# atx/padne

Hardware: AMD Instinct MI355X
Metric: CG solves/s (higher is better)
Workload: dtype f64; 1 GPU; C4 8-layer N=10M: 8-layer jittered triangular Laplacian, 9999392 nodes, via-ring stitched, 1 A source/sink, amg-PCG to rtol 1e-12; n_unknowns=9999391, nnz_per_rank=69955225, rows_per_rank=9999391, parallelism=layer-partitioned x1

## Files before the change

### padne_amd/csrc/amg.hip

```cpp
#include "common.hpp"

#include <functional>
#include <type_traits>
#include <memory>

#include <algorithm>
#include <chrono>
#include <math.h>
#include <stdlib.h>
#include <string.h>

namespace padne {

struct AmgLevel {
    const padne_csr *A = nullptr;
    padne_csr *A_owned = nullptr;
    padne_csr *P = nullptr;
    padne_csr *R = nullptr;
    padne_csr *W = nullptr;
    double lambda = 2.0;
    double jac = 0.0;
    long long n = 0;
    double *b = nullptr, *xa = nullptr, *xb = nullptr, *tmp = nullptr;
    float *b8 = nullptr, *xa8 = nullptr, *xb8 = nullptr, *tmp8 = nullptr;
// ... 27 lines not shown
};

constexpr double kTheta = 0.08;
constexpr double kOmegaNum = 1.5;
constexpr double kChebRatio = 10.0;
constexpr int kLanczosSteps = 8;
constexpr int kMaxLevels = 16;

struct __attribute__((packed, aligned(4))) I4u { int x, y, z, w; };
struct __attribute__((packed, aligned(4))) I2u { int x, y; };
struct __attribute__((packed, aligned(4))) D2u { double x, y; };
struct __attribute__((packed, aligned(4))) L2u { long long x, y; };
__device__ __forceinline__ int4 load_i4_unaligned(const int *p) {
    const I4u v = *reinterpret_cast<const I4u *>(p);
    return make_int4(v.x, v.y, v.z, v.w);
}
__device__ __forceinline__ double2 load_d2_unaligned(const double *p) {
    const D2u v = *reinterpret_cast<const D2u *>(p);
    return make_double2(v.x, v.y);
}

template <int LANES>
__device__ __forceinline__ int scan_incl_lanes(int x) {
    x += __builtin_amdgcn_update_dpp(0, x, 0x111, 0xf, 0xf, false);
    x += __builtin_amdgcn_update_dpp(0, x, 0x112, 0xf, 0xf, false);
    x += __builtin_amdgcn_update_dpp(0, x, 0x114, 0xf, 0xf, false);
    x += __builtin_amdgcn_update_dpp(0, x, 0x118, 0xf, 0xf, false);
    if (LANES >= 32) x += __builtin_amdgcn_update_dpp(0, x, 0x142, 0xa, 0xf, false);
    if (LANES == 64) x += __builtin_amdgcn_update_dpp(0, x, 0x143, 0xc, 0xf, false);
    return x;
}

__device__ __forceinline__ unsigned xcd_bid() {
    const unsigned b = blockIdx.x, per = gridDim.x >> 3;
    if (b >= (per << 3)) return b;
    return (b & 7u) * per + (b >> 3);
}
struct XcdSweep { long long t0, t1, stride; };
__device__ __forceinline__ XcdSweep xcd_sweep(const long long n_tiles, const int waves_per_block, const int w) {
    const unsigned G = gridDim.x;
    const unsigned nslab = (G % kNumXcd == 0) ? kNumXcd : 1;
    const unsigned slab = blockIdx.x % nslab;
    XcdSweep sw;
    const long long s0 = (long long)slab * n_tiles / nslab;
    sw.t1 = (long long)(slab + 1) * n_tiles / nslab;
    sw.t0 = s0 + (long long)(blockIdx.x / nslab) * waves_per_block + w;
    sw.stride = (long long)(G / nslab) * waves_per_block;
    return sw;
}



constexpr unsigned int kMisRoot = 0xffffffffu;
__device__ __forceinline__ unsigned int prio32_of(int i) {
    unsigned int h = (unsigned int)i & 0x7fffffffu;
    h = (h * 0x5bd1e995u) & 0x7fffffffu;
    h ^= h >> 15;
    h = (h * 0x2c1b3c6du) & 0x7fffffffu;
    h ^= h >> 13;
    h = (h * 0x297a2d39u) & 0x7fffffffu;
    h ^= h >> 16;
    return h + 1u;
}

__device__ __forceinline__ bool strong(double a, double di, double dj, double theta2) {
    return a * a * di * dj >= theta2;
}

__device__ __forceinline__ int xw_position(const int4 d, const int run, const int c) {
    int pos = 0;
    if (c >= d.z && c < d.z + run) pos = 2 * run + (c - d.z);
    if (c >= d.y && c < d.y + run) pos = run + (c - d.y);
    if (c >= d.x && c < d.x + run) pos = c - d.x;
    return pos;
}

__global__ __launch_bounds__(256) void strength_mark(int n, int n_wtiles, const int *__restrict__ rowptr,
                                                     const int *__restrict__ cols, const double *__restrict__ vals,
                                                     const double *__restrict__ dinv, double theta2,
                                                     int *__restrict__ scol, double *__restrict__ bound_partial,
                                                     const int4 *__restrict__ xw_desc = nullptr,
                                                     const unsigned char *__restrict__ xw_lidx = nullptr,
                                                     const int xw_run = 0, unsigned char *__restrict__ spos = nullptr,
                                                     float *__restrict__ vals32 = nullptr) {
    constexpr int CH = 512;
    __shared__ unsigned char rid_all[4 * CH];
    __shared__ double pv_all[4 * CH];
    __shared__ double red[4], red2[4];
    const int lane = threadIdx.x & 63, w = threadIdx.x >> 6;
    unsigned char *rid = rid_all + w * CH;
    double *pv = pv_all + w * CH;
    const XcdSweep sw = xcd_sweep(n_wtiles, 4, w);
    double my_max = 0.0, my_plain = 0.0;
    for (long long wt = sw.t0; wt < sw.t1; wt += sw.stride) {
        const int row0 = (int)wt * 64;
        const int row1 = min(row0 + 64, n);
        const int r = row0 + lane;
        int rs = 0, re = 0;
        double di = 0.0;
        if (r < row1) {
            rs = rowptr[r];
            re = rowptr[r + 1];
            di = dinv[r];
        }
        const int k0 = __shfl(rs, 0, 64);
        const int k1 = __shfl(re, row1 - row0 - 1, 64);
        double dF = r < row1 ? 1.0 / di : 1.0, off_strong = 0.0, off_all = 0.0, abs_all = 0.0;
        int4 dsc = make_int4(0, 0, 0, 0);
        if (spos != nullptr) dsc = xw_desc[wt];
        const bool windowed = spos != nullptr && dsc.w != 0;
        const int self_pos = windowed ? xw_position(dsc, xw_run, r) : 0;
        for (int base = k0; base < k1; base += CH) {
            const int lo = max(rs, base), hi = min(re, base + CH);
            for (int k = lo; k < hi; ++k) rid[k - base] = (unsigned char)lane;
            asm volatile("s_waitcnt lgkmcnt(0)" ::: "memory");
            __builtin_amdgcn_wave_barrier();
#pragma unroll
            for (int q = 0; q < CH / 64; ++q) {
                const int e = base + lane + 64 * q;
                const int rl = e < k1 ? rid[e - base] : 0;
                const double dr = __shfl(di, rl, 64);
                const int sp = __shfl(self_pos, rl, 64);
                if (e < k1) {
                    const int i = row0 + rl;
                    const int c = cols[e];
                    const double v = vals[e];
                    if (vals32 != nullptr) vals32[e] = (float)v;
                    const bool st = c != i && strong(v, dr, dinv[c], theta2);
                    scol[e] = st ? c : i;
                    if (windowed) spos[e] = st ? xw_lidx[e] : (unsigned char)sp;
                    if (bound_partial != nullptr) {
                        rid[e - base] = (unsigned char)(rl | (c == i ? 0x40 : 0) | (st ? 0x80 : 0));
                        pv[e - base] = v;
                    }
                }
            }
            if (bound_partial != nullptr) {
                asm volatile("s_waitcnt lgkmcnt(0)" ::: "memory");
                __builtin_amdgcn_wave_barrier();
                for (int k = lo; k < hi; ++k) {
                    const unsigned char f = rid[k - base];
                    const double v = pv[k - base];
                    abs_all += fabs(v);
                    if (f & 0x40) continue;
                    off_all += fabs(v);
                    if (f & 0x80) off_strong += fabs(v);
                    else dF += v;
                }
            }
            asm volatile("" ::: "memory");
            __builtin_amdgcn_wave_barrier();
        }
        if (bound_partial != nullptr && r < row1) {
            double off = off_strong;
            if (!(dF * di > 0.05)) {
                dF = 1.0 / di;
                off = off_all;
            }
            const double sgm = (off + fabs(dF)) / fabs(dF);
            my_max = sgm > my_max ? sgm : my_max;
            const double plain = abs_all * fabs(di);
            my_plain = plain > my_plain ? plain : my_plain;
        }
    }
    if (bound_partial != nullptr) {
        for (int o = 32; o > 0; o >>= 1) {
            my_max = fmax(my_max, __shfl_down(my_max, o, 64));
            my_plain = fmax(my_plain, __shfl_down(my_plain, o, 64));
        }
        if (lane == 0) {
            red[w] = my_max;
            red2[w] = my_plain;
        }
        __syncthreads();
        if (threadIdx.x == 0) {
            bound_partial[blockIdx.x] = fmax(fmax(red[0], red[1]), fmax(red[2], red[3]));
            bound_partial[kMaxPartials + blockIdx.x] = fmax(fmax(red2[0], red2[1]), fmax(red2[2], red2[3]));
        }
    }
}

template <typename T>
__global__ __launch_bounds__(256) void nbr_max(int n, int n_wtiles, const int *__restrict__ srow,
                                               const int *__restrict__ scol, const T *__restrict__ in,
                                               T *__restrict__ out) {
    constexpr int CH = 512;
    __shared__ T park_all[4 * CH];
    const int lane = threadIdx.x & 63, w = threadIdx.x >> 6;
    T *park = park_all + w * CH;
    const XcdSweep sw = xcd_sweep(n_wtiles, 4, w);
    for (long long wt = sw.t0; wt < sw.t1; wt += sw.stride) {
        const int row0 = (int)wt * 64;
        const int row1 = min(row0 + 64, n);
        const int r = row0 + lane;
        int rs = 0, re = 0;
        T m = 0;
        if (r < row1) {
            rs = srow[r];
            re = srow[r + 1];
            m = in[r];
        }
        const int k0 = __shfl(rs, 0, 64);
        const int k1 = __shfl(re, row1 - row0 - 1, 64);
        for (int base = k0; base < k1; base += CH) {
#pragma unroll
            for (int j = 0; j < CH / 64; ++j) {
                const int e = base + lane + 64 * j;
                park[lane + 64 * j] = (e < k1) ? in[scol[e]] : (T)0;
            }
            asm volatile("s_waitcnt lgkmcnt(0)" ::: "memory");
            __builtin_amdgcn_wave_barrier();
            const int lo = max(rs, base), hi = min(re, base + CH);
            for (int k = lo; k < hi; ++k) {
                const T v = park[k - base];
                m = v > m ? v : m;
            }
            asm volatile("" ::: "memory");
            __builtin_amdgcn_wave_barrier();
        }
        if (r < row1) out[r] = m;
    }
}

template <typename T>
__global__ __launch_bounds__(256) void nbr_max_wpr(int n, const int *__restrict__ srow, const int *__restrict__ scol,
                                                   const T *__restrict__ in, T *__restrict__ out) {
    const int lane = threadIdx.x & 63;
    const long long r = (long long)blockIdx.x * 4 + (threadIdx.x >> 6);
    if (r >= n) return;
    const int rs = srow[r], re = srow[r + 1];
    T m = in[r];
    for (int k = rs + lane; k < re; k += 64) {
        const T v = in[scol[k]];
// ... 714 lines not shown
                    }
                    cols[s0 + b + 1] = c;
                    vals[s0 + b + 1] = v;
                }
            }
            continue;
        }
        for (int e = threadIdx.x; e < n; e += 256) {
            Cs[e] = cols[s0 + e];
            Vs[e] = vals[s0 + e];
        }
        __syncthreads();
        for (int e = threadIdx.x; e < n; e += 256) {
            const int c = Cs[e];
            int rank = 0;
            for (int f = 0; f < n; ++f) rank += Cs[f] < c ? 1 : 0;
            cols[s0 + rank] = c;
            vals[s0 + rank] = Vs[e];
        }
        __syncthreads();
    }
}

__global__ void spgemm_count(int n_rows, const int *__restrict__ xr, const int *__restrict__ xc,
                             const int *__restrict__ yr, const int *__restrict__ ye, int *__restrict__ cnt) {
    const int i = xcd_bid() * blockDim.x + threadIdx.x;
    if (i >= n_rows) return;
    long long c = 0;
    const int k0 = xr[i], k1 = xr[i + 1];
    {
        const int4 ca = load_i4_unaligned(xc + k0), cb = load_i4_unaligned(xc + k0 + 4);
        const int m[8] = {ca.x, ca.y, ca.z, ca.w, cb.x, cb.y, cb.z, cb.w};
        int ln[8];
#pragma unroll
        for (int u = 0; u < 8; ++u) {
            ln[u] = 0;
            if (k0 + u < k1) {
                if (ye == yr + 1) {
                    const I2u be = *reinterpret_cast<const I2u *>(yr + m[u]);
                    ln[u] = be.y - be.x;
                } else {
                    ln[u] = ye[m[u]] - yr[m[u]];
                }
            }
        }
#pragma unroll
        for (int u = 0; u < 8; ++u) c += ln[u];
    }
    for (int k = k0 + 8; k < k1; ++k) {
        const int m = xc[k];
        c += ye[m] - yr[m];
    }
    cnt[i] = c > 2000000000LL ? 2000000000 : (int)c;
}

template <int LPR>
__global__ __launch_bounds__(256) void spgemm_count_lanes(int n_rows, const int *__restrict__ xr, const int *__restrict__ xc,
                                                          const int *__restrict__ yr, const int *__restrict__ ye, int *__restrict__ cnt) {
    const long long tid = (long long)xcd_bid() * blockDim.x + threadIdx.x;
    const long long i = tid / LPR;
    const int l = (int)(tid % LPR);
    long long c = 0;
    if (i < n_rows) {
        const int k0 = xr[i], k1 = xr[i + 1];
        int k = k0 + l;
        for (; k + LPR < k1; k += 2 * LPR) {
            const int m0 = xc[k], m1 = xc[k + LPR];
            const int b0 = yr[m0], e0 = ye[m0], b1 = yr[m1], e1 = ye[m1];
            c += (e0 - b0) + (e1 - b1);
        }
        if (k < k1) {
            const int m0 = xc[k];
            c += ye[m0] - yr[m0];
        }
    }
#pragma unroll
    for (int d = 1; d < LPR; d <<= 1) c += __shfl_xor(c, d, 64);
    if (i < n_rows && l == 0) cnt[i] = c > 2000000000LL ? 2000000000 : (int)c;
}

__global__ void spgemm_rows(int n_rows, const int *__restrict__ xr, const int *__restrict__ xc,
                            const double *__restrict__ xv, const int *__restrict__ yr, const int *__restrict__ yc,
                            const double *__restrict__ yv, const int *__restrict__ ye, const int ycs, const int *__restrict__ slot_ptr,
                            long long *__restrict__ key, double *__restrict__ val, int *__restrict__ row_len) {
    const int i = blockIdx.x * blockDim.x + threadIdx.x;
    if (i >= n_rows) return;
    long long *K = key + slot_ptr[i];
    double *V = val + slot_ptr[i];
    int m = 0;
    for (int k = xr[i]; k < xr[i + 1]; ++k) {
        const int mid = xc[k];
        const double a = xv[k];
        for (int q = yr[mid]; q < ye[mid]; ++q) {
            const long long c = (long long)yc[(long long)q * ycs] << 32;
            const double v = a * yv[q];
            int lo = 0, hi = m;
            while (lo < hi) {
                const int h = (lo + hi) >> 1;
                if (K[h] < c) lo = h + 1; else hi = h;
            }
            if (lo < m && K[lo] == c) {
                V[lo] += v;
            } else {
                for (int t = m; t > lo; --t) {
                    K[t] = K[t - 1];
                    V[t] = V[t - 1];
                }
                K[lo] = c;
                V[lo] = v;
                ++m;
            }
        }
    }
    row_len[i] = m;
}

template <int CAP, int KC, int QC, int YCS>
__global__ __launch_bounds__(128) void spgemm_rows_lds_pipe(int n_rows, const int *__restrict__ xr, const int *__restrict__ xc,
                                                            const double *__restrict__ xv, const int *__restrict__ yr,
                                                            const int *__restrict__ yc, const double *__restrict__ yv,
                                                            const int *__restrict__ ye, const int *__restrict__ slot_ptr,
                                                            long long *__restrict__ key, double *__restrict__ val,
                                                            int *__restrict__ row_len, int *__restrict__ begin) {
    static_assert(CAP % 2 == 0, "keys are kept in pairs");
    __shared__ int2 Kc[CAP / 2][128];
    __shared__ double Vc[CAP][128];
    const int t = threadIdx.x;
    const int i = xcd_bid() * 128 + t;
    const bool live = i < n_rows;
    if (begin == nullptr && !live) return;
    int m = 0;
    bool overflow = false;
#pragma unroll
    for (int u = 0; u < CAP / 2; ++u) Kc[u][t] = make_int2(-1, -1);
    auto insert = [&](const bool act, const int c, const double v) {
        int pos = -1;
#pragma unroll
        for (int u = 0; u < CAP; u += 2) {
            if (__all(u >= m)) break;
            const int2 kk = Kc[u >> 1][t];
            pos = kk.x == c ? u : pos;
            pos = kk.y == c ? u + 1 : pos;
        }
        if (act && !overflow) {
            const bool found = pos >= 0;
            if (!found && m == CAP) {
                overflow = true;
            } else {
                const int p = found ? pos : m;
                const double base = found ? Vc[p][t] : -0.0;
                Vc[p][t] = base + v;
                if (!found) {
                    reinterpret_cast<int *>(&Kc[p >> 1][t])[p & 1] = c;
                    ++m;
                }
            }
        }
    };
    const int x0 = live ? xr[i] : 0, x1 = live ? xr[i + 1] : 0;
    for (int kb = x0; kb < x1 && !overflow; kb += KC) {
        const int nk = min(KC, x1 - kb);
        int mid[KC], ys[KC], ln[KC];
        double a[KC];
        static_assert(KC % 4 == 1 && QC == 4, "the loads below are written for 4 k + 1 entries of X and rows of Y read four at a time");
#pragma unroll
        for (int u = 0; u < KC - 1; u += 4) {
            const I4u c4 = *reinterpret_cast<const I4u *>(xc + kb + u);
            mid[u] = c4.x; mid[u + 1] = c4.y; mid[u + 2] = c4.z; mid[u + 3] = c4.w;
            const D2u v0 = *reinterpret_cast<const D2u *>(xv + kb + u), v1 = *reinterpret_cast<const D2u *>(xv + kb + u + 2);
            a[u] = v0.x; a[u + 1] = v0.y; a[u + 2] = v1.x; a[u + 3] = v1.y;
        }
        mid[KC - 1] = xc[kb + KC - 1];
        a[KC - 1] = xv[kb + KC - 1];
#pragma unroll
        for (int u = 0; u < KC; ++u) {
            mid[u] = u < nk ? mid[u] : 0;
            if (ye == yr + 1) {
                const I2u be = *reinterpret_cast<const I2u *>(yr + mid[u]);
                ys[u] = be.x;
                ln[u] = u < nk ? be.y - be.x : 0;
            } else {
                ys[u] = yr[mid[u]];
                ln[u] = u < nk ? ye[mid[u]] - ys[u] : 0;
            }
        }
        int cb[2][QC];
        double vb[2][QC];
        auto fetch = [&](const int u, int (&c)[QC], double (&v)[QC]) {
            if (YCS == 1) {
                const I4u c4 = *reinterpret_cast<const I4u *>(yc + ys[u]);
                c[0] = c4.x; c[1] = c4.y; c[2] = c4.z; c[3] = c4.w;
            } else {
                const L2u k0 = *reinterpret_cast<const L2u *>(reinterpret_cast<const long long *>(yc) + ys[u]);
                const L2u k1 = *reinterpret_cast<const L2u *>(reinterpret_cast<const long long *>(yc) + ys[u] + 2);
                c[0] = (int)k0.x; c[1] = (int)k0.y; c[2] = (int)k1.x; c[3] = (int)k1.y;
            }
            const D2u v0 = *reinterpret_cast<const D2u *>(yv + ys[u]), v1 = *reinterpret_cast<const D2u *>(yv + ys[u] + 2);
            v[0] = v0.x; v[1] = v0.y; v[2] = v1.x; v[3] = v1.y;
        };
        fetch(0, cb[0], vb[0]);
#pragma unroll
        for (int u = 0; u < KC; ++u) {
            if (u + 1 < KC) fetch(u + 1, cb[(u + 1) & 1], vb[(u + 1) & 1]);
#pragma unroll
            for (int w = 0; w < QC; ++w)
                if (__any(w < ln[u])) insert(w < ln[u], cb[u & 1][w], a[u] * vb[u & 1][w]);
            for (int q = QC; q < ln[u] && !overflow; ++q)
                insert(true, yc[(long long)(ys[u] + q) * YCS], a[u] * yv[ys[u] + q]);
        }
    }
    int place = live ? slot_ptr[i] : 0;
    if (begin != nullptr) {
        const int lane = t & 63;
        const int tile0 = i - lane, tile1 = min(tile0 + 64, n_rows);
        const int len = (live && !overflow) ? m : 0;
        const int bound = (live && overflow) ? slot_ptr[i + 1] - slot_ptr[i] : 0;
        const int incl = scan_incl_lanes<64>(len);
        const int bound_incl = scan_incl_lanes<64>(bound);
        const int back = __builtin_amdgcn_readlane(bound_incl, 63) - bound_incl + bound;
        if (tile0 < n_rows) {
            const int r_begin = slot_ptr[tile0], r_end = slot_ptr[tile1];
            place = overflow ? r_end - back : r_begin + (incl - len);
        }
        if (live) begin[i] = place;
    }
    if (!live) return;
    if (overflow) {
        row_len[i] = -1;
        return;
    }
    long long *K = key + place;
    double *V = val + place;
    int kr[CAP];
#pragma unroll
    for (int u = 0; u < CAP; u += 2) {
        const int2 kk = Kc[u >> 1][t];
        kr[u] = u < m ? kk.x : 2147483647;
        kr[u + 1] = u + 1 < m ? kk.y : 2147483647;
    }
#pragma unroll
    for (int u = 0; u < CAP; ++u) {
        if (__all(u >= m)) break;
        int rank = 0;
#pragma unroll
        for (int w = 0; w < CAP; ++w) rank += kr[w] < kr[u] ? 1 : 0;
        if (u < m) {
            K[rank] = (long long)kr[u] << 32;
            V[rank] = Vc[u][t];
        }
    }
    row_len[i] = m;
}

template <int CAPP, int HT, int LANES>
struct SpgemmRowLds {
    using Mask = typename std::conditional<LANES == 64, unsigned long long, unsigned>::type;
    int ht[HT];
    int hidx[HT];
    int dk[HT / 2];
    Mask mask[HT / 2];
    double pvb[LANES];
    double xs[LANES];
    int ys[LANES];
    int offc[LANES];
    unsigned long long bits[CAPP / 64];
};

template <int CAPP, int HT, int LANES>
__device__ __forceinline__ int spgemm_row_by_masks(SpgemmRowLds<CAPP, HT, LANES> &S, const int sl, const int sub,
                                                   const bool has_row, const int nx, const int len, const int ystart,
                                                   const double a, const int *__restrict__ yc, const double *__restrict__ yv,
                                                   const int ycs, long long *__restrict__ K, double *__restrict__ V) {
    using Mask = typename SpgemmRowLds<CAPP, HT, LANES>::Mask;
    static_assert(CAPP % 64 == 0 && CAPP / 64 <= LANES && 64 % LANES == 0, "bits of the product offsets");
    constexpr int NC = (HT / 2 + LANES - 1) / LANES;
    constexpr int EMPTY = -1;
    const unsigned long long sub_mask = (LANES == 64 ? ~0ull : ((1ull << LANES) - 1ull));
    const int shift = sub * LANES;
    const unsigned long long below = (1ull << sl) - 1ull;
    static_assert(LANES == 16 || LANES == 32 || LANES == 64, "the scan below");
    const int incl = scan_incl_lanes<LANES>(len);
    const int np = LANES == 64   ? __builtin_amdgcn_readlane(incl, 63)
                   : LANES == 32 ? (sub != 0 ? __builtin_amdgcn_readlane(incl, 63) : __builtin_amdgcn_readlane(incl, 31))
                                 : __builtin_amdgcn_update_dpp(0, incl, 0x15F, 0xf, 0xf, false);
    const bool live = has_row && nx <= LANES && np <= CAPP;
    const unsigned long long have = (__ballot(live && len > 0) >> shift) & sub_mask;
    if (live) {
        for (int h = sl; h < HT; h += LANES) S.ht[h] = EMPTY;
        for (int h = sl; h < HT / 2; h += LANES) S.mask[h] = (Mask)0;
        if (sl < CAPP / 64) S.bits[sl] = 0ull;
        asm volatile("s_waitcnt lgkmcnt(0)" ::: "memory");
        if (len > 0) {
            const int pos = __popcll(have & below);
            const int o = incl - len;
            S.offc[pos] = o;
            S.ys[pos] = ystart;
            S.xs[pos] = a;
            atomicOr(&S.bits[o >> 6], 1ull << (o & 63));
        }
    }
    asm volatile("s_waitcnt lgkmcnt(0)" ::: "memory");
    __builtin_amdgcn_wave_barrier();
    int np_w = live ? np : 0;
    if (LANES == 64) {
        np_w = __builtin_amdgcn_readfirstlane(np_w);
    } else {
        int m = 0;
#pragma unroll
        for (int g = 0; g < 64 / LANES; ++g) m = max(m, __builtin_amdgcn_readlane(np_w, g * LANES));
        np_w = m;
    }
    int cnt = 0, pre = 0;
    bool overflow = false;
// ... 5 lines not shown
        const bool mine = live && p < np;
        unsigned long long word = 0ull;
        if (live && base < np) word = S.bits[base >> 6];
        int c = 0;
        if (mine) {
            const int kk = pre + __popcll(word & (~0ull >> (63 - (p & 63)))) - 1;
            const int q = S.ys[kk] + (p - S.offc[kk]);
            c = yc[(long long)q * ycs];
            S.pvb[sl] = S.xs[kk] * yv[q];
        }
        if (((base + LANES) & 63) == 0) pre += __popcll(word);
        bool pending = mine;
        unsigned h = ((unsigned)c * 2654435761u) >> 7;
        int idx = -1;
        for (int round = 0; __any(pending); ++round) {
            if (round == HT) {
                overflow = overflow || pending;
                break;
            }
            h &= (HT - 1);
            int old = EMPTY - 1;
            if (pending) old = atomicCAS(&S.ht[h], EMPTY, c);
            const bool won = old == EMPTY;
            const unsigned long long wm = (__ballot(won) >> shift) & sub_mask;
            if (won) {
                idx = cnt + __popcll(wm & below);
                S.hidx[h] = idx;
                if (idx < HT / 2) S.dk[idx] = c;
            }
            cnt += __popcll(wm);
            asm volatile("" ::: "memory");
            const bool hit = pending && old == c;
            if (hit) idx = S.hidx[h];
            pending = pending && !won && !hit;
            ++h;
        }
        if (mine && idx >= 0 && idx < HT / 2) atomicOr(&S.mask[idx], (Mask)1 << sl);
        asm volatile("s_waitcnt lgkmcnt(0)" ::: "memory");
        __builtin_amdgcn_wave_barrier();
#pragma unroll
        for (int u = 0; u < NC; ++u) {
            const int j = sl + u * LANES;
            if (live && j < cnt && j < HT / 2) {
                Mask m = S.mask[j];
                if (m != (Mask)0) {
                    S.mask[j] = (Mask)0;
                    do {
                        const int b = (LANES == 64 ? __ffsll((long long)m) : __ffs((int)m)) - 1;
                        acc[u] += S.pvb[b];
                        m &= m - (Mask)1;
                    } while (m != (Mask)0);
                }
            }
        }
        asm volatile("s_waitcnt lgkmcnt(0)" ::: "memory");
        __builtin_amdgcn_wave_barrier();
    }
    const bool any_overflow = ((__ballot(overflow) >> shift) & sub_mask) != 0ull;
    const int nd = cnt;
    const bool ok = live && !any_overflow && nd <= HT / 2;
#pragma unroll
    for (int u = 0; u < NC; ++u) {
        const int j = sl + u * LANES;
        if (ok && j < nd) {
            const int kq = S.dk[j];
            int rank = 0;
            for (int t = 0; t < nd; ++t) rank += S.dk[t] < kq ? 1 : 0;
            K[rank] = (long long)kq << 32;
            V[rank] = acc[u];
        }
    }
    asm volatile("s_waitcnt lgkmcnt(0)" ::: "memory");
    __builtin_amdgcn_wave_barrier();
    return ok ? nd : -1;
}

template <int CAPP, int HT, int LANES, bool LIST>
__global__ __launch_bounds__(256) void spgemm_rows_lanes(int n_rows, const int *__restrict__ xr, const int *__restrict__ xc,
                                                         const double *__restrict__ xv, const int *__restrict__ yr,
                                                         const int *__restrict__ yc, const double *__restrict__ yv, const int *__restrict__ ye, const int ycs,
                                                         const int *__restrict__ slot_ptr, long long *__restrict__ key,
                                                         double *__restrict__ val, int *__restrict__ row_len,
                                                         const int *__restrict__ row_list = nullptr,
                                                         const int *__restrict__ list_count = nullptr) {
    constexpr int G = 256 / LANES;
    __shared__ SpgemmRowLds<CAPP, HT, LANES> s_rows[G];
    const int lane = threadIdx.x & 63;
    const int sl = lane % LANES, sub = lane / LANES, g = threadIdx.x / LANES;
    constexpr bool listed = LIST;
    int t_l, t_end, stride;
    if (listed) {
        t_end = *list_count;
        t_l = (int)blockIdx.x * G + g;
        stride = (int)gridDim.x * G;
    } else {
        const int nslab = (gridDim.x % kNumXcd == 0) ? kNumXcd : 1;
        const int slab = blockIdx.x % nslab;
        t_end = (int)((long long)(slab + 1) * n_rows / nslab);
        t_l = (int)((long long)slab * n_rows / nslab) + (int)(blockIdx.x / nslab) * G + g;
        stride = (int)(gridDim.x / nslab) * G;
    }
    if (t_l > t_end) t_l = t_end;
    int row_l = -1;
    int row_a = -1, x0_a = 0, x1_a = 0, len_a = -1;
    int row_b = -1, x0_b = 0, x1_b = 0, len_b = -1, mid_b = 0;
    double a_b = 0.0;
    int row_c = -1, nx_c = 0, len_c = -1, ys_c = 0, ye_c = 0, place_c = 0;
    double a_c = 0.0;
    auto advance = [&]() {
        const int nx_b = x1_b - x0_b;
        row_c = row_b; nx_c = nx_b; len_c = len_b; a_c = a_b; ys_c = 0; ye_c = 0; place_c = 0;
        if (row_b >= 0) {
            place_c = slot_ptr[row_b];
            if (nx_b <= LANES && sl < nx_b) {
                ys_c = yr[mid_b];
                ye_c = ye[mid_b];
            }
        }
        const int nx_a = x1_a - x0_a;
        row_b = row_a; x0_b = x0_a; x1_b = x1_a; len_b = len_a; mid_b = 0; a_b = 0.0;
        if (row_a >= 0 && nx_a <= LANES && sl < nx_a) {
            mid_b = xc[x0_a + sl];
            a_b = xv[x0_a + sl];
        }
        row_a = row_l; x0_a = 0; x1_a = 0; len_a = -1;
        if (row_a >= 0) {
            x0_a = xr[row_a];
            x1_a = xr[row_a + 1];
            if (listed) len_a = row_len[row_a];
        }
        row_l = -1;
        if (t_l < t_end) row_l = listed ? row_list[t_l] : t_l;
        t_l = t_l < t_end - stride ? t_l + stride : t_end;
    };
    advance();
    advance();
    advance();
    advance();
    while (__any(row_c >= 0)) {
        const int i = row_c;
        const bool has_row = i >= 0 && !(listed && len_c >= 0);
        const int nx = nx_c, ystart = ys_c, len = ye_c - ys_c, place = place_c;
        const double a = a_c;
        advance();
        const int nd = spgemm_row_by_masks<CAPP, HT, LANES>(s_rows[g], sl, sub, has_row, nx, len, ystart, a, yc, yv, ycs,
                                                            key + place, val + place);
        if (has_row && sl == 0) row_len[i] = nd;
    }
}

__global__ __launch_bounds__(256) void spgemm_rows_dense(int n_cols, const int *__restrict__ xr, const int *__restrict__ xc,
                                                         const double *__restrict__ xv, const int *__restrict__ yr,
                                                         const int *__restrict__ yc, const double *__restrict__ yv, const int *__restrict__ ye, const int ycs,
                                                         const int *__restrict__ slot_ptr, long long *__restrict__ key,
                                                         double *__restrict__ val, int *__restrict__ row_len,
                                                         const int only_pending, const int *__restrict__ row_list = nullptr,
                                                         const int *__restrict__ list_count = nullptr) {
    extern __shared__ double acc_and_flag[];
    double *acc = acc_and_flag;
    unsigned char *hit = (unsigned char *)(acc + n_cols);
    __shared__ int wave_cnt[4];
    const int n_turns = row_list != nullptr ? *list_count : 1;
    for (int turn = row_list != nullptr ? (int)blockIdx.x : 0; turn < n_turns; turn += row_list != nullptr ? (int)gridDim.x : 1) {
    const int i = row_list != nullptr ? row_list[turn] : (int)blockIdx.x;
    if (only_pending && row_len[i] >= 0) continue;
    __syncthreads();
    for (int c = threadIdx.x; c < n_cols; c += 256) {
        acc[c] = 0.0;
        hit[c] = 0;
    }
    __syncthreads();
    for (int k = xr[i]; k < xr[i + 1]; ++k) {
        const int mid = xc[k];
        const double a = xv[k];
        for (int q = yr[mid] + threadIdx.x; q < ye[mid]; q += 256) {
            const int c = yc[(long long)q * ycs];
            acc[c] += a * yv[q];
            hit[c] = 1;
        }
        __syncthreads();
    }
    long long *K = key + slot_ptr[i];
    double *V = val + slot_ptr[i];
    int base = 0;
    const int lane = threadIdx.x & 63, w = threadIdx.x >> 6;
    for (int c0 = 0; c0 < n_cols; c0 += 256) {
        const int c = c0 + threadIdx.x;
        const bool on = c < n_cols && hit[c];
        const unsigned long long bal = __ballot(on);
        if (lane == 0) wave_cnt[w] = __popcll(bal);
        __syncthreads();
        int off = base;
        for (int u = 0; u < w; ++u) off += wave_cnt[u];
        const int total = wave_cnt[0] + wave_cnt[1] + wave_cnt[2] + wave_cnt[3];
        if (on) {
            const int pos = off + __popcll(bal & ((1ull << lane) - 1ull));
            K[pos] = (long long)c << 32;
            V[pos] = acc[c];
        }
        base += total;
        __syncthreads();
    }
    if (threadIdx.x == 0) row_len[i] = base;
    }
}

__global__ __launch_bounds__(256) void collect_pending_rows(int n, const int *__restrict__ row_len, int *__restrict__ list,
                                                            int *__restrict__ count) {
    const int i = blockIdx.x * 256 + threadIdx.x;
    const bool pend = i < n && row_len[i] < 0;
    __shared__ int wave_cnt[4], block_base;
    const unsigned long long mask = __ballot(pend);
    const int lane = threadIdx.x & 63, w = threadIdx.x >> 6;
    if (lane == 0) wave_cnt[w] = __popcll(mask);
    __syncthreads();
    if (threadIdx.x == 0) {
        const int t = wave_cnt[0] + wave_cnt[1] + wave_cnt[2] + wave_cnt[3];
        block_base = t ? atomicAdd(count, t) : 0;
    }
    __syncthreads();
    int base = block_base;
    for (int q = 0; q < w; ++q) base += wave_cnt[q];
    if (pend) list[base + __popcll(mask & ((1ull << lane) - 1ull))] = i;
}

__global__ void spgemm_rows_redo(int n_rows, const int *__restrict__ xr, const int *__restrict__ xc,
                                 const double *__restrict__ xv, const int *__restrict__ yr, const int *__restrict__ yc,
                                 const double *__restrict__ yv, const int *__restrict__ ye, const int ycs, const int *__restrict__ slot_ptr,
                                 long long *__restrict__ key, double *__restrict__ val, int *__restrict__ row_len) {
    const int i = blockIdx.x * blockDim.x + threadIdx.x;
    if (i >= n_rows || row_len[i] >= 0) return;
    long long *K = key + slot_ptr[i];
    double *V = val + slot_ptr[i];
    int m = 0;
    for (int k = xr[i]; k < xr[i + 1]; ++k) {
        const int mid = xc[k];
        const double a = xv[k];
        for (int q = yr[mid]; q < ye[mid]; ++q) {
            const long long c = (long long)yc[(long long)q * ycs] << 32;
            const double v = a * yv[q];
            int lo = 0, hi = m;
            while (lo < hi) {
                const int h = (lo + hi) >> 1;
                if (K[h] < c) lo = h + 1; else hi = h;
            }
            if (lo < m && K[lo] == c) {
                V[lo] += v;
            } else {
                for (int u = m; u > lo; --u) {
                    K[u] = K[u - 1];
                    V[u] = V[u - 1];
                }
                K[lo] = c;
                V[lo] = v;
                ++m;
            }
        }
    }
    row_len[i] = m;
}

__global__ void dense_from_csr(int n, const int *__restrict__ rowptr, const int *__restrict__ cols,
                               const double *__restrict__ vals, double *__restrict__ W) {
    const int i = blockIdx.x;
    for (int c = threadIdx.x; c < n; c += blockDim.x) W[(size_t)i * n + c] = 0.0;
    __syncthreads();
    for (int k = rowptr[i] + threadIdx.x; k < rowptr[i + 1]; k += blockDim.x) W[(size_t)i * n + cols[k]] = vals[k];
}

constexpr int kGjBlock = 16;
constexpr int kGjStrip = 32;
__device__ __forceinline__ double Rsel(const double (&R)[kGjBlock], int a) {
    double v = 0.0;
#pragma unroll
    for (int b = 0; b < kGjBlock; ++b) v = (a == b) ? R[b] : v;
    return v;
}
__device__ __forceinline__ void gj_invert_block16(double (&dd)[4], const int lane) {
    const int eb = lane & 15, ea0 = lane >> 4;
#pragma unroll
    for (int p = 0; p < kGjBlock; ++p) {
        const double dpp = __shfl(dd[p >> 2], ((p & 3) << 4) | p, 64);
        const double drow = __shfl(dd[p >> 2], ((p & 3) << 4) | eb, 64);
        double dcol[4];
#pragma unroll
        for (int q = 0; q < 4; ++q) dcol[q] = __shfl(dd[q], (lane & 48) | p, 64);
        double inv = __builtin_amdgcn_rcp(dpp);
        inv = fma(inv, fma(-dpp, inv, 1.0), inv);
        inv = fma(inv, fma(-dpp, inv, 1.0), inv);
        const double rp = drow * inv;
#pragma unroll
        for (int q = 0; q < 4; ++q) {
            const int ea = ea0 + 4 * q;
            const double cp = dcol[q];
            dd[q] = (ea == p) ? (eb == p ? inv : rp) : (eb == p ? -cp * inv : dd[q] - cp * rp);
        }
    }
}

template <bool kFull>
__global__ __launch_bounds__(256) void gj_block_step(int n, int k0, const double *__restrict__ in, double *__restrict__ out) {
    static_assert(kGjBlock == 16, "the pivot block inversion below maps a 16 x 16 block onto one wave");
    __shared__ __attribute__((aligned(16))) double Dinv[kGjBlock][kGjBlock];
    __shared__ __attribute__((aligned(16))) double Lcol[kGjStrip][kGjBlock];
    const int bs = kFull ? kGjBlock : min(kGjBlock, n - k0);
    const int r0 = blockIdx.y * kGjStrip;
    const int c = blockIdx.x * blockDim.x + threadIdx.x;
    const bool live = c < n;
    const bool pivot_col = c >= k0 && c < k0 + bs;
    double P[kGjBlock], V[kGjStrip];
#pragma unroll
    for (int b = 0; b < kGjBlock; ++b) P[b] = (live && !pivot_col && b < bs) ? in[(size_t)(k0 + b) * n + c] : 0.0;
#pragma unroll
    for (int q = 0; q < kGjStrip; ++q) {
        const int i = r0 + q;
        V[q] = (live && i < n && !pivot_col) ? in[(size_t)i * n + c] : 0.0;
    }
    for (int t = threadIdx.x; t < kGjStrip * kGjBlock; t += 256) {
        const int i = r0 + t / kGjBlock, b = t % kGjBlock;
        Lcol[t / kGjBlock][b] = (i < n && (kFull || b < bs)) ? in[(size_t)i * n + k0 + b] : 0.0;
    }
    if (threadIdx.x < 64) {
        const int lane = threadIdx.x, eb = lane & 15, ea0 = lane >> 4;
        double dd[4];
#pragma unroll
        for (int q = 0; q < 4; ++q) {
            const int ea = ea0 + 4 * q;
            dd[q] = (ea < bs && eb < bs) ? in[(size_t)(k0 + ea) * n + k0 + eb] : (ea == eb ? 1.0 : 0.0);
        }
        gj_invert_block16(dd, lane);
#pragma unroll
        for (int q = 0; q < 4; ++q) Dinv[ea0 + 4 * q][eb] = dd[q];
    }
    __syncthreads();
    if (!live) return;
    double R[kGjBlock];
    if (pivot_col) {
#pragma unroll
        for (int a = 0; a < kGjBlock; ++a) R[a] = Dinv[a][c - k0];
    } else {
#pragma unroll
        for (int a = 0; a < kGjBlock; ++a) {
// ... 358 lines not shown
}

__global__ __launch_bounds__(256) void fold_range_kernel(const double *__restrict__ mins, const double *__restrict__ maxs, int g,
                                                         double *__restrict__ out2) {
    __shared__ double lo_s[256], hi_s[256];
    double lo = 1e300, hi = 0.0;
    for (int q = threadIdx.x; q < g; q += 256) {
        const double a = mins[q], b = maxs[q];
        lo = a < lo ? a : lo;
        if (b > hi || !(b == b)) hi = b;
    }
    lo_s[threadIdx.x] = lo;
    hi_s[threadIdx.x] = hi;
    __syncthreads();
    for (int off = 128; off > 0; off >>= 1) {
        if ((int)threadIdx.x < off) {
            const double a = lo_s[threadIdx.x + off], b = hi_s[threadIdx.x + off];
            if (a < lo_s[threadIdx.x]) lo_s[threadIdx.x] = a;
            if (!(hi_s[threadIdx.x] == hi_s[threadIdx.x])) {
            } else if (b > hi_s[threadIdx.x] || !(b == b)) {
                hi_s[threadIdx.x] = b;
            }
        }
        __syncthreads();
    }
    if (threadIdx.x == 0) {
        out2[0] = lo_s[0];
        out2[1] = hi_s[0];
    }
}


static bool amg_verbose();

__global__ __launch_bounds__(256) void fold_max2_kernel(const double *__restrict__ a, const double *__restrict__ b, int g,
                                                        double *__restrict__ out2) {
    __shared__ double red[2][256];
    double ma = 0.0, mb = 0.0;
    for (int q = threadIdx.x; q < g; q += 256) {
        ma = a[q] > ma ? a[q] : ma;
        if (b != nullptr) mb = b[q] > mb ? b[q] : mb;
    }
    red[0][threadIdx.x] = ma;
    red[1][threadIdx.x] = mb;
    __syncthreads();
    for (int off = 128; off > 0; off >>= 1) {
        if ((int)threadIdx.x < off) {
            red[0][threadIdx.x] = fmax(red[0][threadIdx.x], red[0][threadIdx.x + off]);
            red[1][threadIdx.x] = fmax(red[1][threadIdx.x], red[1][threadIdx.x + off]);
        }
        __syncthreads();
    }
    if (threadIdx.x == 0) {
        out2[0] = red[0][0];
        out2[1] = red[1][0];
    }
}

static int gershgorin(padne_ctx *ctx, const padne_csr *A, double *lambda, bool filtered = false) {
    const int g = (int)std::min<long long>((A->n_rows + 255) / 256, 1024);
    double *part = ctx->partials + 6 * kMaxPartials;
    if (filtered)
        hipLaunchKernelGGL(gershgorin_filtered_kernel, dim3(g > 0 ? g : 1), dim3(256), 0, ctx->stream, (int)A->n_rows,
                           A->rowptr, A->cols, A->vals, A->dinv, kTheta * kTheta, part);
    else
        hipLaunchKernelGGL(gershgorin_kernel, dim3(g > 0 ? g : 1), dim3(256), 0, ctx->stream, (int)A->n_rows, A->rowptr,
                           A->vals, A->dinv, part);
    hipLaunchKernelGGL(fold_max2_kernel, dim3(1), dim3(256), 0, ctx->stream, (const double *)part, (const double *)nullptr,
                       g > 0 ? g : 1, part + kMaxPartials - 2);
    PADNE_HIP_CHECK(hipGetLastError());
    double h[2] = {0.0, 0.0};
    PADNE_TRY(read_back(ctx, part + kMaxPartials - 2, sizeof(h), h));
    double m = h[0];
    if (!(m > 0.0) || !(m < 1e6)) m = 2.0;
    *lambda = m;
    return PADNE_OK;
}

static int aggregate(padne_ctx *ctx, Scratch &sc, const padne_csr *A, int **agg_out, int *n_agg, double *lambda_f = nullptr,
                     double *lambda_plain = nullptr, unsigned char **spos_out = nullptr, int **scol_out = nullptr,
                     float *vals32_out = nullptr, signed char **state_out = nullptr) {
    hipStream_t s = ctx->stream;
    const int n = (int)A->n_rows;
    const double theta2 = kTheta * kTheta;
    signed char *state = nullptr;
    unsigned int *w0 = nullptr, *w1 = nullptr, *w2 = nullptr;
    int *flag = nullptr, *scan = nullptr, *agg0 = nullptr, *agg1 = nullptr, *counter = nullptr;
    PADNE_TRY(sc.alloc(&state, (size_t)n));
    PADNE_TRY(sc.alloc(&w0, (size_t)n));
    PADNE_TRY(sc.alloc(&w1, (size_t)n));
    PADNE_TRY(sc.alloc(&w2, (size_t)n));
    PADNE_TRY(sc.alloc(&flag, (size_t)n + 1));
    PADNE_TRY(sc.alloc(&scan, (size_t)n + 1));
    PADNE_TRY(sc.alloc(&agg0, (size_t)n));
    PADNE_TRY(sc.alloc(&agg1, (size_t)n));
    constexpr int kMaxRounds = 256;
    PADNE_TRY(sc.alloc(&counter, (size_t)2 * kMaxRounds + 4));
    const dim3 g(nblk(n)), b(256);
    const int *srow = A->rowptr;
    int *scol = nullptr;
    PADNE_TRY(sc.alloc(&scol, (size_t)(A->nnz > 0 ? A->nnz : 1)));
    const int n_wt = (n + 63) / 64;
    int gm_x = std::min(2048, (n_wt + 3) / 4 > 0 ? (n_wt + 3) / 4 : 1);
    if (gm_x >= kNumXcd) gm_x -= gm_x % kNumXcd;
    const dim3 gm((unsigned)gm_x);
    double *bound_part = lambda_f != nullptr ? ctx->partials + 6 * kMaxPartials : nullptr;
    double *bound2 = nullptr;
    if (lambda_f != nullptr) PADNE_TRY(sc.alloc(&bound2, 2));
    const bool xw = A->xw_state == 1 && A->xw_run <= 85;
    unsigned char *spos = nullptr;
    if (xw) {
        PADNE_TRY(sc.alloc(&spos, (size_t)A->nnz + kPadNnz));
    }
    static_assert(kPadNnz >= 2 * kMaxRounds + 4, "one grid for everything the start clears");
    hipLaunchKernelGGL(mis_init_words, dim3(nblk(std::max(n, kPadNnz))), b, 0, s, n, w0, state, counter, 2 * kMaxRounds + 4,
                       spos != nullptr ? spos + A->nnz : (unsigned char *)nullptr, kPadNnz);
    hipLaunchKernelGGL(strength_mark, gm, b, 0, s, n, n_wt, A->rowptr, A->cols, A->vals, A->dinv, theta2, scol, bound_part,
                       xw ? A->xw_desc : (const int4 *)nullptr, xw ? (const unsigned char *)A->xw_lidx : (const unsigned char *)nullptr,
                       xw ? A->xw_run : 0, spos, vals32_out);
    PADNE_HIP_CHECK(hipGetLastError());
    const bool long_rows = !xw && n <= 65536 && A->nnz >= 24LL * n;
    auto launch_round = [&](int *open_counter) {
        if (xw) {
            hipLaunchKernelGGL((nbr_max_xw<unsigned int, false>), gm, b, 0, s, n, n_wt, srow, scol, spos, A->xw_desc, A->xw_run,
                               (const unsigned int *)w0, w1, (unsigned int *)nullptr, (signed char *)nullptr, (int *)nullptr);
            hipLaunchKernelGGL((nbr_max_xw<unsigned int, true>), gm, b, 0, s, n, n_wt, srow, scol, spos, A->xw_desc, A->xw_run,
                               (const unsigned int *)w1, (unsigned int *)nullptr, w0, state, open_counter);
        } else if (long_rows) {
            hipLaunchKernelGGL(nbr_max_wpr<unsigned int>, dim3((unsigned)((n + 3) / 4)), b, 0, s, n, srow, (const int *)scol,
                               (const unsigned int *)w0, w1);
            hipLaunchKernelGGL(nbr_max_wpr<unsigned int>, dim3((unsigned)((n + 3) / 4)), b, 0, s, n, srow, (const int *)scol,
                               (const unsigned int *)w1, w2);
            hipLaunchKernelGGL(mis_decide, dim3(std::min<unsigned>(g.x, 1024u)), b, 0, s, n, w0, w2, state, open_counter);
        } else {
            hipLaunchKernelGGL(nbr_max<unsigned int>, gm, b, 0, s, n, n_wt, srow, scol, w0, w1);
            hipLaunchKernelGGL(nbr_max<unsigned int>, gm, b, 0, s, n, n_wt, srow, scol, w1, w2);
            hipLaunchKernelGGL(mis_decide, dim3(std::min<unsigned>(g.x, 1024u)), b, 0, s, n, w0, w2, state, open_counter);
        }
    };
    if (lambda_f != nullptr)
        hipLaunchKernelGGL(fold_max2_kernel, dim3(1), dim3(256), 0, s, (const double *)bound_part,
                           (const double *)(bound_part + kMaxPartials), (int)gm.x, bound2);
    double h_bound2[2] = {0.0, 0.0};
    bool bound_pending = lambda_f != nullptr;
    auto count_back = [&](const int *dev_count, int *host_count) -> int {
        if (!bound_pending) return read_back(ctx, dev_count, sizeof(int), host_count);
        bound_pending = false;
        return read_back2(ctx, dev_count, sizeof(int), host_count, bound2, sizeof(h_bound2), h_bound2);
    };
    int open_count = n;
    int round = 0;
    const bool compact_ok = A->nnz <= 16LL * n;
    const int full_batch = n > 200000 ? 1 : 4;
    while (round < kMaxRounds && open_count > 0 && (!compact_ok || round < 2 || open_count > n / 8)) {
        const int reps = (round == 0 && compact_ok && full_batch < 2) ? 2 : full_batch;
        for (int rep = 0; rep < reps && round < kMaxRounds; ++rep, ++round) {
            launch_round(counter + round);
        }
        PADNE_HIP_CHECK(hipGetLastError());
        PADNE_TRY(count_back(counter + round - 1, &open_count));
    }
    if (open_count > 0) {
        int *list_a = (int *)w1, *list_b = (int *)w2;
        unsigned int *m2 = nullptr;
        PADNE_TRY(sc.alloc(&m2, (size_t)open_count));
        int *counters = counter + kMaxRounds;
        hipLaunchKernelGGL(mis_collect_open, dim3(std::min<unsigned>(g.x, 1024u)), b, 0, s, n, state, list_a, counters);
        PADNE_HIP_CHECK(hipGetLastError());
        int cnt = open_count, cur = 0;
        while (cur + 1 < kMaxRounds && cnt > 0) {
            if (cnt <= kMisTailCap) {
                hipLaunchKernelGGL(mis_tail_rounds, dim3(1), dim3(1024), 0, s, (const int *)(counters + cur), list_a, list_b, srow,
                                   (const int *)scol, w0, state, m2, counters + cur + 1, kMaxRounds - cur - 1);
                PADNE_HIP_CHECK(hipGetLastError());
                ++cur;
                round += kMaxRounds;
                PADNE_TRY(count_back(counters + cur, &cnt));
                break;
            }
            const dim3 gl(nblk(cnt));
            const int batch = 4;
            for (int rep = 0; rep < batch && cur + 1 < kMaxRounds; ++rep, ++round) {
                hipLaunchKernelGGL(mis_two_hop_max, dim3(nblk((long long)cnt * kHopLanes)), b, 0, s, counters + cur, list_a, srow, scol, w0, m2);
                hipLaunchKernelGGL(mis_decide_list, gl, b, 0, s, counters + cur, list_a, m2, w0, state, list_b, counters + cur + 1);
                std::swap(list_a, list_b);
                ++cur;
            }
            PADNE_HIP_CHECK(hipGetLastError());
            PADNE_TRY(count_back(counters + cur, &cnt));
        }
        open_count = cnt;
    }
    PADNE_REQUIRE(open_count == 0, "independent-set rounds did not terminate");
    if (lambda_f != nullptr) {
        if (bound_pending) PADNE_TRY(read_back(ctx, bound2, sizeof(h_bound2), h_bound2));
        double m = h_bound2[0], mp = h_bound2[1];
        if (!(m > 0.0) || !(m < 1e6)) m = 2.0;
        if (!(mp > 0.0) || !(mp < 1e6)) mp = 2.0;
        *lambda_f = m;
        if (lambda_plain != nullptr) *lambda_plain = mp;
    }
    hipLaunchKernelGGL(flag_state, g, b, 0, s, n, state, flag, 1);
    ScanTicket t_roots, t_single;
    long long h_roots[2] = {0, 0}, h_single[2] = {0, 0};
    PADNE_TRY(scan_i32_begin(ctx, flag, scan, n, &t_roots, true));
    hipLaunchKernelGGL(agg_from_roots, g, b, 0, s, n, state, scan, agg0);
    hipLaunchKernelGGL(agg_join, g, b, 0, s, n, srow, scol, A->vals, agg0, agg1);
    hipLaunchKernelGGL(agg_join, g, b, 0, s, n, srow, scol, A->vals, agg1, agg0);
    hipLaunchKernelGGL(flag_unaggregated, g, b, 0, s, n, agg0, flag);
    int rc_scan = scan_i32_begin(ctx, flag, scan, n, &t_single, true);
    if (rc_scan == PADNE_OK && t_roots.bs != nullptr)
        hipLaunchKernelGGL(agg_singletons, g, b, 0, s, n, scan, (const long long *)(t_roots.bs + t_roots.nb), agg0);
    const int rc_roots = scan_i32_end(ctx, &t_roots, h_roots);
    if (rc_scan == PADNE_OK) rc_scan = scan_i32_end(ctx, &t_single, h_single);
    PADNE_TRY(rc_roots);
    PADNE_TRY(rc_scan);
    PADNE_HIP_CHECK(hipGetLastError());
    const long long n_roots = h_roots[0], n_single = h_single[0];
    PADNE_REQUIRE(n_roots >= 0 && n_single >= 0 && n_roots + n_single < 2147483647LL, "aggregate count out of range");
    *agg_out = agg0;
    *n_agg = (int)(n_roots + n_single);
    if (spos_out != nullptr) *spos_out = spos;
    if (scol_out != nullptr) *scol_out = scol;
    if (state_out != nullptr) *state_out = state;
    return PADNE_OK;
}

template <int CAP>
__global__ __launch_bounds__(128) void prolong_rows_lds(int n, const int *__restrict__ rowptr, const int *__restrict__ cols,
                                                        const double *__restrict__ vals, const double *__restrict__ dinv,
                                                        double theta2, double omega, const int *__restrict__ agg,
                                                        const int *__restrict__ slot_ptr, long long *__restrict__ key,
                                                        double *__restrict__ val, int *__restrict__ row_len) {
    static_assert(CAP % 2 == 0, "keys are kept in pairs");
    __shared__ int2 Kc[CAP / 2][128];
    __shared__ double Vc[CAP][128];
    const int t = threadIdx.x;
    const int i = blockIdx.x * 128 + t;
    if (i >= n) return;
    const double di = dinv[i];
    double dF = 1.0 / di;
    const int k0 = rowptr[i], k1 = rowptr[i + 1];
    for (int kb = k0; kb < k1; kb += 8) {
        const int4 ca = load_i4_unaligned(cols + kb), cb = load_i4_unaligned(cols + kb + 4);
        const double2 v0 = load_d2_unaligned(vals + kb), v1 = load_d2_unaligned(vals + kb + 2),
                      v2 = load_d2_unaligned(vals + kb + 4), v3 = load_d2_unaligned(vals + kb + 6);
        const int j[8] = {ca.x, ca.y, ca.z, ca.w, cb.x, cb.y, cb.z, cb.w};
        const double a[8] = {v0.x, v0.y, v1.x, v1.y, v2.x, v2.y, v3.x, v3.y};
        double dj[8];
#pragma unroll
        for (int u = 0; u < 8; ++u) dj[u] = kb + u < k1 ? dinv[j[u]] : 1.0;
#pragma unroll
        for (int u = 0; u < 8; ++u)
            if (kb + u < k1 && j[u] != i && !strong(a[u], di, dj[u], theta2)) dF += a[u];
    }
    const bool keep_all = !(dF * di > 0.05);
    if (keep_all) dF = 1.0 / di;
    const double w = -omega / dF;
    const int ai = agg[i];
#pragma unroll
    for (int u = 0; u < CAP / 2; ++u) Kc[u][t] = make_int2(-1, -1);
    int m = 1;
    reinterpret_cast<int *>(&Kc[0][t])[0] = ai;
    Vc[0][t] = 1.0;
    bool overflow = false;
    auto insert = [&](const bool act, const int c, const double v) {
        int pos = -1;
#pragma unroll
        for (int u = 0; u < CAP; u += 2) {
            if (__all(u >= m)) break;
            const int2 kk = Kc[u >> 1][t];
            pos = kk.x == c ? u : pos;
            pos = kk.y == c ? u + 1 : pos;
        }
        if (act && !overflow) {
            const bool found = pos >= 0;
            if (!found && m == CAP) {
                overflow = true;
            } else {
                const int p = found ? pos : m;
                const double base = found ? Vc[p][t] : -0.0;
                Vc[p][t] = base + v;
                if (!found) {
                    reinterpret_cast<int *>(&Kc[p >> 1][t])[p & 1] = c;
                    ++m;
                }
            }
        }
    };
    for (int kb = k0; kb < k1 && !overflow; kb += 8) {
        const int4 ca = load_i4_unaligned(cols + kb), cb = load_i4_unaligned(cols + kb + 4);
        const double2 v0 = load_d2_unaligned(vals + kb), v1 = load_d2_unaligned(vals + kb + 2),
                      v2 = load_d2_unaligned(vals + kb + 4), v3 = load_d2_unaligned(vals + kb + 6);
        const int j[8] = {ca.x, ca.y, ca.z, ca.w, cb.x, cb.y, cb.z, cb.w};
        const double a[8] = {v0.x, v0.y, v1.x, v1.y, v2.x, v2.y, v3.x, v3.y};
        double dj[8];
        int aj[8];
#pragma unroll
        for (int u = 0; u < 8; ++u) {
            const bool on = kb + u < k1;
            dj[u] = on ? dinv[j[u]] : 1.0;
            aj[u] = on ? agg[j[u]] : 0;
        }
#pragma unroll
        for (int u = 0; u < 8; ++u) {
            const bool on = kb + u < k1;
            const bool diag = on && j[u] == i;
            const bool act = on && (diag || keep_all || strong(a[u], di, dj[u], theta2));
            if (__any(act)) insert(act, diag ? ai : aj[u], diag ? -omega : w * a[u]);
        }
    }
    if (overflow) {
        row_len[i] = -1;
        return;
    }
    int o = 0;
    for (int u = 0; u < m; ++u) {
        if (Vc[u][t] != 0.0) ++o;
        else reinterpret_cast<int *>(&Kc[u >> 1][t])[u & 1] = 0x7fffffff;
    }
    long long *K = key + slot_ptr[i];
    double *V = val + slot_ptr[i];
    for (int u = 0; u < CAP; ++u) {
        if (__all(u >= m)) break;
        const int ku = u < m ? reinterpret_cast<const int *>(&Kc[u >> 1][t])[u & 1] : 0x7fffffff;
        int rank = 0;
        for (int q = 0; q < CAP; q += 2) {
            if (__all(q >= m)) break;
            const int2 kk = Kc[q >> 1][t];
            rank += (q < m && kk.x < ku) ? 1 : 0;
            rank += (q + 1 < m && kk.y < ku) ? 1 : 0;
        }
        if (ku != 0x7fffffff) {
            K[rank] = (long long)ku << 32;
            V[rank] = Vc[u][t];
        }
    }
    row_len[i] = o;
}

constexpr int kPxSlots = 14;
constexpr int kPxChunk = 640;
template <int SLOTS>
__device__ __forceinline__ int prolong_row_merge(const bool live, const int w, const int rs, const int re, const int k0, const int self,
                                                 const bool windowed, const double di, const double omega, const int r,
                                                 const unsigned char (*Ls)[kPxChunk], const unsigned char (*Ss)[kPxChunk],
                                                 const double (*Vs)[kPxChunk], const int (*As)[3 * 88],
                                                 const int *__restrict__ cols, const int *__restrict__ scol,
                                                 const double *__restrict__ vals, const int *__restrict__ agg,
                                                 int (&c)[SLOTS], double (&sum)[SLOTS], bool (&keep)[SLOTS]) {
    const int len = live ? re - rs : 0;
    int el[SLOTS - 1], es[SLOTS - 1];
    double ev[SLOTS - 1];
    double dF = 1.0 / di;
#pragma unroll
    for (int k = 0; k < SLOTS - 1; ++k) {
        const bool in = k < len;
        el[k] = in ? (windowed ? (int)Ls[w][rs - k0 + k] : cols[rs + k]) : -1;
        es[k] = in ? (windowed ? (int)Ss[w][rs - k0 + k] : scol[rs + k]) : -1;
        ev[k] = in ? (windowed ? Vs[w][rs - k0 + k] : vals[rs + k]) : 0.0;
        if (in && el[k] != self && es[k] == self) dF += ev[k];
    }
    const bool keep_all = !(dF * di > 0.05);
    if (keep_all) dF = 1.0 / di;
    const double wgt = -omega / dF;
    const int ai = live ? (windowed ? As[w][self] : agg[r]) : 0;
    double v[SLOTS];
    c[0] = ai;
    v[0] = 1.0;
#pragma unroll
    for (int k = 0; k < SLOTS - 1; ++k) {
        const bool in = k < len;
        const bool diag = in && el[k] == self;
        const bool used = in && (diag || keep_all || es[k] != self);
        int cj = 0x7fffffff;
        if (used && !diag) cj = windowed ? As[w][el[k]] : agg[el[k]];
        c[k + 1] = diag ? ai : cj;
        v[k + 1] = diag ? -omega : (used ? wgt * ev[k] : 0.0);
    }
    int o = 0;
#pragma unroll
    for (int k = 0; k < SLOTS; ++k) {
        bool first = c[k] != 0x7fffffff;
#pragma unroll
        for (int j = 0; j < k; ++j) first = first && c[j] != c[k];
        double t = v[k];
#pragma unroll
        for (int j = k + 1; j < SLOTS; ++j) t = c[j] == c[k] ? t + v[j] : t;
        sum[k] = t;
        keep[k] = live && first && t != 0.0;
        o += keep[k] ? 1 : 0;
    }
    return o;
}

template <int SLOTS>
// ... 31 lines not shown
        int rs = 0, re = 0;
        double di = 1.0;
        if (r < row1) {
            rs = rowptr[r];
            re = rowptr[r + 1];
            di = dinv[r];
        }
        const int4 d = xw_desc[wt];
        const int k0 = __shfl(rs, 0, 64);
        const int k1 = __shfl(re, row1 - row0 - 1, 64);
        const bool too_long = re - rs > kPxSlots - 1;
        if (__any(too_long)) {
            if (r < row1) row_len[r] = -1;
            continue;
        }
        const bool windowed = d.w != 0 && k1 - k0 <= kPxChunk;
        if (windowed) {
            const int st[3] = {d.x, d.y, d.z};
#pragma unroll
            for (int q = 0; q < 3; ++q) {
                const int a = st[q] + lane, b = st[q] + 64 + lane;
                As[w][q * run + lane] = a < n ? agg[a] : 0;
                if (lane < run - 64) As[w][q * run + 64 + lane] = b < n ? agg[b] : 0;
            }
            for (int e = k0 + lane; e < k1; e += 64) {
                Ls[w][e - k0] = lidx[e];
                Ss[w][e - k0] = spos[e];
                Vs[w][e - k0] = vals[e];
            }
        }
        asm volatile("s_waitcnt vmcnt(0) lgkmcnt(0)" ::: "memory");
        __builtin_amdgcn_wave_barrier();
        const int self = windowed ? xw_position(d, run, r) : r;
        const int tile_base = k0 + row0;
        if (__all(re - rs <= 9)) {
            int c[10];
            double sum[10];
            bool keep[10];
            const int o = prolong_row_merge<10>(r < row1, w, rs, re, k0, self, windowed, di, omega, r, Ls, Ss, Vs, As, cols, scol, vals, agg, c, sum, keep);
            const int before = scan_incl_lanes<64>(o) - o;
            if (r < row1) row_len[r] = o;
            prolong_row_store<10>(c, sum, keep, tile_base + before, st_cols, st_vals);
        } else {
            int c[kPxSlots];
            double sum[kPxSlots];
            bool keep[kPxSlots];
            const int o = prolong_row_merge<kPxSlots>(r < row1, w, rs, re, k0, self, windowed, di, omega, r, Ls, Ss, Vs, As, cols, scol, vals, agg, c, sum, keep);
            const int before = scan_incl_lanes<64>(o) - o;
            if (r < row1) row_len[r] = o;
            prolong_row_store<kPxSlots>(c, sum, keep, tile_base + before, st_cols, st_vals);
        }
        asm volatile("" ::: "memory");
        __builtin_amdgcn_wave_barrier();
    }
}

__global__ __launch_bounds__(256) void prolong_unstage(int n, int n_wtiles, const int *__restrict__ a_rowptr,
                                                       const int *__restrict__ rowptr, const int *__restrict__ st_cols,
                                                       const double *__restrict__ st_vals, int *__restrict__ cols,
                                                       double *__restrict__ vals) {
    const int lane = threadIdx.x & 63, w = threadIdx.x >> 6;
    const XcdSweep sw = xcd_sweep(n_wtiles, 4, w);
    for (long long wt = sw.t0; wt < sw.t1; wt += sw.stride) {
        const int row0 = (int)wt * 64;
        const int row1 = min(row0 + 64, n);
        const int src = a_rowptr[row0] + row0;
        const int d0 = rowptr[row0], d1 = rowptr[row1];
        for (int k = lane; k < d1 - d0; k += 64) {
            cols[d0 + k] = st_cols[src + k];
            vals[d0 + k] = st_vals[src + k];
        }
    }
}

__global__ void prolong_redo_flag(int n, const int *__restrict__ row_len, int *__restrict__ any) {
    const int i = blockIdx.x * blockDim.x + threadIdx.x;
    if (i < n && row_len[i] < 0) atomicExch(any, 1);
}

static int build_prolongator(padne_ctx *ctx, const padne_csr *A, const int *agg, int n_agg, double omega,
                             padne_csr **P, const unsigned char *spos = nullptr, const int *scol = nullptr) {
    hipStream_t s = ctx->stream;
    const int n = (int)A->n_rows;
    Scratch sc(ctx);
    if (spos != nullptr && scol != nullptr && A->xw_state == 1 && A->xw_run <= 85 && n > 0 &&
        (long long)A->nnz + (long long)n < 2147483647LL) {
        int *row_len = nullptr, *rowptr_tmp = nullptr, *st_cols = nullptr;
        double *st_vals = nullptr;
        PADNE_TRY(sc.alloc(&row_len, (size_t)n + 1));
        PADNE_TRY(sc.alloc(&rowptr_tmp, (size_t)n + 1));
        PADNE_TRY(sc.alloc(&st_cols, (size_t)A->nnz + (size_t)n));
        PADNE_TRY(sc.alloc(&st_vals, (size_t)A->nnz + (size_t)n));
        const int n_wt = (n + 63) / 64;
        const dim3 g((unsigned)std::min((n_wt + 3) / 4, 8192)), b(256);
        hipLaunchKernelGGL(prolong_rows_xw, g, b, 0, s, n, n_wt, A->rowptr, A->cols, A->vals, A->dinv, scol,
                           (const unsigned char *)A->xw_lidx, spos, A->xw_desc, A->xw_run, omega, agg, row_len, st_cols, st_vals);
        PADNE_HIP_CHECK(hipGetLastError());
        int64_t nnz = 0;
        bool h_gave_up = false;
        PADNE_TRY(exclusive_scan_i32_flagged(ctx, row_len, rowptr_tmp, n, &nnz, &h_gave_up));
        if (!h_gave_up) {
            padne_csr *m = nullptr;
            PADNE_TRY(csr_alloc(ctx, n, n_agg, nnz, &m));
            PADNE_HIP_CHECK(hipMemcpyAsync(m->rowptr, rowptr_tmp, sizeof(int32_t) * (size_t)(n + 1), hipMemcpyDeviceToDevice, s));
            hipLaunchKernelGGL(prolong_unstage, dim3((unsigned)std::min((n_wt + 3) / 4, 2048)), b, 0, s, n, n_wt, A->rowptr,
                               (const int *)rowptr_tmp, (const int *)st_cols, (const double *)st_vals, m->cols, m->vals);
            PADNE_HIP_CHECK(hipGetLastError());
            *P = m;
            return PADNE_OK;
        }
    }
    const size_t n_slots = (size_t)A->nnz + (size_t)n;
    int *slot_ptr = nullptr, *row_len = nullptr, *any = nullptr;
    long long *key = nullptr;
    double *val = nullptr;
    PADNE_TRY(sc.alloc(&slot_ptr, (size_t)n + 1));
    PADNE_TRY(sc.alloc(&row_len, (size_t)n + 1));
    PADNE_TRY(sc.alloc(&any, 1));
    PADNE_TRY(sc.alloc(&key, n_slots));
    PADNE_TRY(sc.alloc(&val, n_slots));
    PADNE_HIP_CHECK(hipMemsetAsync(any, 0, sizeof(int), s));
    hipLaunchKernelGGL(prolong_slot_ptr, dim3(nblk((long long)n + 1)), dim3(256), 0, s, n, A->rowptr, slot_ptr);
    hipLaunchKernelGGL(prolong_rows_lds<24>, dim3(nblk(n, 128)), dim3(128), 0, s, n, A->rowptr, A->cols, A->vals, A->dinv,
                       kTheta * kTheta, omega, agg, slot_ptr, key, val, row_len);
    hipLaunchKernelGGL(prolong_redo_flag, dim3(nblk(n)), dim3(256), 0, s, n, row_len, any);
    PADNE_HIP_CHECK(hipGetLastError());
    int h_any = 0;
    PADNE_TRY(read_back(ctx, any, sizeof(int), &h_any));
    if (h_any) {
        hipLaunchKernelGGL(prolong_fill, dim3(nblk((long long)n + 1)), dim3(256), 0, s, n, A->rowptr, A->cols, A->vals,
                           A->dinv, kTheta * kTheta, omega, agg, slot_ptr, key, val);
        PADNE_HIP_CHECK(hipGetLastError());
        PADNE_TRY(merge_slots_generic(ctx, n, slot_ptr, key, val, row_len));
    }
    return csr_from_slots(ctx, n, n_agg, slot_ptr, key, val, row_len, P);
}

static int transpose(padne_ctx *ctx, const padne_csr *M, padne_csr **T) {
    hipStream_t s = ctx->stream;
    Scratch sc(ctx);
    const long long nc = M->n_cols;
    PADNE_REQUIRE(M->n_rows < 2147483647LL && nc < 2147483647LL, "transpose of a matrix beyond 32-bit indices");
    int *zeroed = nullptr, *long_list = nullptr, *pairs = nullptr;
    const size_t n_zero = 3 * (size_t)nc + 4;
    PADNE_TRY(sc.alloc(&zeroed, n_zero));
    PADNE_TRY(sc.alloc(&long_list, (size_t)nc + 1));
    PADNE_TRY(sc.alloc(&pairs, (size_t)nc * kTpK + 4));
    int *cnt = zeroed, *cursor = zeroed + nc + 1, *npairs = cursor + nc, *n_long = npairs + nc;
    padne_csr *m = nullptr;
    PADNE_TRY(csr_alloc(ctx, nc, M->n_rows, M->nnz, &m));
    const int all_cursors = ctx->opt.force_transpose_cursors ? 1 : 0;
    hipError_t e = hipMemsetAsync(zeroed, 0, sizeof(int) * n_zero, s);
    if (e == hipSuccess && M->n_rows > 0)
        hipLaunchKernelGGL(transpose_count_pairs, dim3(nblk(M->n_rows)), dim3(256), 0, s, (int)M->n_rows, M->rowptr, M->cols, cnt,
                           npairs, pairs, all_cursors);
    int rc = e == hipSuccess ? exclusive_scan_i32_async(ctx, cnt, m->rowptr, nc) : PADNE_E_HIP;
    if (rc == PADNE_OK && e == hipSuccess && M->n_rows > 0) {
        hipLaunchKernelGGL(transpose_fill_ordered, dim3(nblk(M->n_rows)), dim3(256), 0, s, (int)M->n_rows, M->rowptr, M->cols,
                           M->vals, (const int *)m->rowptr, (const int *)npairs, (const int *)pairs, cursor, m->cols, m->vals,
                           all_cursors);
        const long long n_chunks = (nc + kSegRows - 1) / kSegRows;
        unsigned g = (unsigned)std::min<long long>((n_chunks + 3) / 4, 8192);
        if (g >= (unsigned)kNumXcd) g -= g % kNumXcd;
        hipLaunchKernelGGL(sort_csr_rows_seg, dim3(g > 0 ? g : 1), dim3(256), 0, s, (int)nc, (const int *)m->rowptr, m->cols, m->vals,
                           n_long, long_list, (const int *)npairs);
        hipLaunchKernelGGL(sort_listed_csr_rows, dim3(2048), dim3(256), 0, s, (const int *)n_long, (const int *)long_list,
                           (const int *)m->rowptr, m->cols, m->vals);
        e = hipGetLastError();
    }
    if (rc == PADNE_OK && e != hipSuccess) {
        set_error("transpose failed: %s", hipGetErrorString(e));
        rc = PADNE_E_HIP;
    }
    if (rc != PADNE_OK) {
        padne_csr_destroy(m);
        return rc;
    }
    *T = m;
    return PADNE_OK;
}

struct SlotRows {
    padne_ctx *ctx = nullptr;
    long long n_rows = 0, n_cols = 0, n_slots = 0;
    int *begin = nullptr, *end = nullptr;
    long long *key = nullptr;
    double *val = nullptr;
    bool valid = false;
    ~SlotRows() { release(); }
    void release() {
        if (ctx != nullptr) {
            pool_free(ctx, begin);
            pool_free(ctx, end);
            pool_free(ctx, key);
            pool_free(ctx, val);
        }
        begin = end = nullptr;
        key = nullptr;
        val = nullptr;
        valid = false;
    }
};

__global__ void slot_row_ends(int n, const int *__restrict__ slot_ptr, const int *__restrict__ row_len, int *__restrict__ end) {
    const int i = blockIdx.x * blockDim.x + threadIdx.x;
    if (i < n) end[i] = slot_ptr[i] + row_len[i];
}

static int spgemm(padne_ctx *ctx, const padne_csr *X, const padne_csr *Y, padne_csr **C, const SlotRows *y_slots = nullptr,
                  SlotRows *keep_slots = nullptr, const std::function<int()> *while_counting = nullptr,
                  const std::function<int()> *while_multiplying = nullptr) {
    const int *y_begin = y_slots != nullptr ? y_slots->begin : Y->rowptr;
    const int *y_end = y_slots != nullptr ? y_slots->end : Y->rowptr + 1;
    const int *y_cols = y_slots != nullptr ? (const int *)y_slots->key + 1 : Y->cols;
    const double *y_vals = y_slots != nullptr ? y_slots->val : Y->vals;
    const int y_cs = y_slots != nullptr ? 2 : 1;
    hipStream_t s = ctx->stream;
    Scratch sc(ctx);
    const int n = (int)X->n_rows;
    int *cnt = nullptr, *slot_ptr = nullptr, *row_len = nullptr;
    PADNE_TRY(sc.alloc(&cnt, (size_t)n + 1));
    PADNE_TRY(sc.alloc(&slot_ptr, (size_t)n + 1));
    PADNE_TRY(sc.alloc(&row_len, (size_t)n + 1));
    if (n > 0) {
        const double x_avg = (double)X->nnz / (double)n;
        if (x_avg > 48.0)
            hipLaunchKernelGGL((spgemm_count_lanes<32>), dim3(nblk((long long)n * 32)), dim3(256), 0, s, n, X->rowptr, X->cols, y_begin, y_end, cnt);
        else if (x_avg > 16.0)
            hipLaunchKernelGGL((spgemm_count_lanes<8>), dim3(nblk((long long)n * 8)), dim3(256), 0, s, n, X->rowptr, X->cols, y_begin, y_end, cnt);
        else
            hipLaunchKernelGGL(spgemm_count, dim3(nblk(n)), dim3(256), 0, s, n, X->rowptr, X->cols, y_begin, y_end, cnt);
    }
    PADNE_HIP_CHECK(hipGetLastError());
    int64_t n_slots = 0;
    int rc_scan = PADNE_OK;
    {
        ScanTicket ticket;
        long long h[2] = {0, 0};
        PADNE_TRY(scan_i32_begin(ctx, cnt, slot_ptr, n, &ticket, true));
        const int rc_cb = while_counting != nullptr ? (*while_counting)() : PADNE_OK;
        rc_scan = scan_i32_end(ctx, &ticket, h);
        PADNE_TRY(rc_cb);
        if (rc_scan == PADNE_OK) {
            if (h[0] < 0 || h[1] != 0) {
                set_error("scan of negative counts");
                rc_scan = PADNE_E_INVALID;
            } else if (h[0] >= 2147483647LL) {
                set_error("%lld entries exceed the 32-bit index space", h[0]);
                rc_scan = PADNE_E_TOOLARGE;
            }
            n_slots = h[0];
        }
    }
    const long long split_limit = ctx->opt.force_spgemm_split;
    if ((rc_scan == PADNE_E_TOOLARGE || (rc_scan == PADNE_OK && split_limit > 0 && n_slots > split_limit)) && n >= 2) {
        sc.release();
        const int h = n / 2;
        padne_csr top = *X, bottom = *X;
        top.n_rows = h;
        bottom.n_rows = n - h;
        bottom.rowptr = X->rowptr + h;
        top.nnz = bottom.nnz = 0;
        top.amg = bottom.amg = nullptr;
        if (amg_verbose()) fprintf(stderr, "[amg]   spgemm %lld rows: %lld product slots, split in two\n", (long long)n, (long long)n_slots);
        padne_csr *Ct = nullptr, *Cb = nullptr;
        int rc = spgemm(ctx, &top, Y, &Ct, y_slots);
        if (rc == PADNE_OK) rc = spgemm(ctx, &bottom, Y, &Cb, y_slots);
        if (rc == PADNE_OK) rc = csr_vstack(ctx, Ct, Cb, Y->n_cols, C);
        if (Ct) padne_csr_destroy(Ct);
        if (Cb) padne_csr_destroy(Cb);
        return rc;
    }
    PADNE_TRY(rc_scan);
    if (amg_verbose()) fprintf(stderr, "[amg]   spgemm %lld rows, %lld product slots\n", (long long)n, (long long)n_slots);
    long long *key = nullptr;
    double *val = nullptr;
    int *row_begin = nullptr;
    PADNE_TRY(sc.alloc(&key, (size_t)n_slots + 4));
    PADNE_TRY(sc.alloc(&val, (size_t)n_slots + 4));
    if (n > 0) {
        const double avg = (double)n_slots / (double)n;
        const size_t dense_lds = (size_t)Y->n_cols * 9 + 16;
        if (avg > 256.0 && dense_lds <= 150 * 1024) {
            (void)hipFuncSetAttribute((const void *)spgemm_rows_dense, hipFuncAttributeMaxDynamicSharedMemorySize,
                                      (int)dense_lds);
            hipLaunchKernelGGL(spgemm_rows_dense, dim3(n), dim3(256), dense_lds, s, (int)Y->n_cols, X->rowptr, X->cols,
                               X->vals, y_begin, y_cols, y_vals, y_end, y_cs, slot_ptr, key, val, row_len, 0);
        } else if (avg <= 24.0) {
            {
                PADNE_TRY(sc.alloc(&row_begin, (size_t)n + 1));
                if (y_cs == 1)
                    hipLaunchKernelGGL((spgemm_rows_lds_pipe<12, 9, 4, 1>), dim3(nblk(n, 128)), dim3(128), 0, s, n, X->rowptr, X->cols,
                                       X->vals, y_begin, y_cols, y_vals, y_end, slot_ptr, key, val, row_len, row_begin);
                else
                    hipLaunchKernelGGL((spgemm_rows_lds_pipe<12, 9, 4, 2>), dim3(nblk(n, 128)), dim3(128), 0, s, n, X->rowptr, X->cols,
                                       X->vals, y_begin, y_cols, y_vals, y_end, slot_ptr, key, val, row_len, row_begin);
            }
            {
                const int *place = row_begin != nullptr ? row_begin : slot_ptr;
                int *pend = nullptr, *pend_count = nullptr;
                PADNE_TRY(sc.alloc(&pend, (size_t)n));
                PADNE_TRY(sc.alloc(&pend_count, 1));
                PADNE_HIP_CHECK(hipMemsetAsync(pend_count, 0, sizeof(int), s));
                hipLaunchKernelGGL(collect_pending_rows, dim3(nblk(n)), dim3(256), 0, s, n, (const int *)row_len, pend, pend_count);
                hipLaunchKernelGGL((spgemm_rows_lanes<1024, 512, 64, true>), dim3(256), dim3(256), 0, s, n, X->rowptr, X->cols, X->vals, y_begin,
                                   y_cols, y_vals, y_end, y_cs, place, key, val, row_len, (const int *)pend, (const int *)pend_count);
                hipLaunchKernelGGL(spgemm_rows_redo, dim3(nblk(n, 128)), dim3(128), 0, s, n, X->rowptr, X->cols, X->vals,
                                   y_begin, y_cols, y_vals, y_end, y_cs, place, key, val, row_len);
            }
        } else if (avg <= 256.0) {
            const unsigned gw = (unsigned)std::min<long long>(((long long)n + 3) / 4, 16384);
            const unsigned gl = std::min(gw, 4096u);
            int *pend = nullptr, *pend_count = nullptr;
            PADNE_TRY(sc.alloc(&pend, (size_t)n));
            PADNE_TRY(sc.alloc(&pend_count, 1));
            PADNE_HIP_CHECK(hipMemsetAsync(pend_count, 0, sizeof(int), s));
            if (avg <= 110.0) {
                const double x_avg = (double)X->nnz / (double)n;
                if (x_avg > 0.0 && x_avg <= 14.0 && avg <= 48.0) {
                    unsigned gs = (unsigned)std::min<long long>(((long long)n + 15) / 16, 16384);
                    hipLaunchKernelGGL((spgemm_rows_lanes<128, 32, 16, false>), dim3(gs), dim3(256), 0, s, n, X->rowptr, X->cols, X->vals,
                                       y_begin, y_cols, y_vals, y_end, y_cs, slot_ptr, key, val, row_len);
                } else {
                    unsigned gs = (unsigned)std::min<long long>(((long long)n + 7) / 8, 16384);
                    hipLaunchKernelGGL((spgemm_rows_lanes<256, 64, 32, false>), dim3(gs), dim3(256), 0, s, n, X->rowptr, X->cols, X->vals,
                                       y_begin, y_cols, y_vals, y_end, y_cs, slot_ptr, key, val, row_len);
                }
                hipLaunchKernelGGL(collect_pending_rows, dim3(nblk(n)), dim3(256), 0, s, n, (const int *)row_len, pend, pend_count);
                hipLaunchKernelGGL((spgemm_rows_lanes<256, 128, 64, true>), dim3(gl), dim3(256), 0, s, n, X->rowptr, X->cols, X->vals,
                                   y_begin, y_cols, y_vals, y_end, y_cs, slot_ptr, key, val, row_len, (const int *)pend,
                                   (const int *)pend_count);
            } else {
                hipLaunchKernelGGL((spgemm_rows_lanes<512, 256, 64, false>), dim3(gw), dim3(256), 0, s, n, X->rowptr, X->cols, X->vals,
                                   y_begin, y_cols, y_vals, y_end, y_cs, slot_ptr, key, val, row_len);
                hipLaunchKernelGGL(collect_pending_rows, dim3(nblk(n)), dim3(256), 0, s, n, (const int *)row_len, pend, pend_count);
            }
            hipLaunchKernelGGL((spgemm_rows_lanes<1024, 512, 64, true>), dim3(std::min(gl, 1024u)), dim3(256), 0, s, n, X->rowptr, X->cols,
                               X->vals, y_begin, y_cols, y_vals, y_end, y_cs, slot_ptr, key, val, row_len, (const int *)pend,
                               (const int *)pend_count);
            if (dense_lds <= 150 * 1024) {
                (void)hipFuncSetAttribute((const void *)spgemm_rows_dense, hipFuncAttributeMaxDynamicSharedMemorySize,
                                          (int)dense_lds);
                hipLaunchKernelGGL(spgemm_rows_dense, dim3(std::min(n, 1024)), dim3(256), dense_lds, s, (int)Y->n_cols, X->rowptr, X->cols,
                                   X->vals, y_begin, y_cols, y_vals, y_end, y_cs, slot_ptr, key, val, row_len, 1, (const int *)pend,
                                   (const int *)pend_count);
            }
            hipLaunchKernelGGL(spgemm_rows_redo, dim3(nblk(n, 128)), dim3(128), 0, s, n, X->rowptr, X->cols, X->vals,
                               y_begin, y_cols, y_vals, y_end, y_cs, slot_ptr, key, val, row_len);
        } else {
            hipLaunchKernelGGL(spgemm_rows, dim3(nblk(n, 128)), dim3(128), 0, s, n, X->rowptr, X->cols, X->vals,
                               y_begin, y_cols, y_vals, y_end, y_cs, slot_ptr, key, val, row_len);
        }
    }
    PADNE_HIP_CHECK(hipGetLastError());
    if (while_multiplying != nullptr && keep_slots != nullptr) PADNE_TRY((*while_multiplying)());
    if (keep_slots != nullptr) {
        keep_slots->release();
        int *end = (int *)pool_alloc(ctx, sizeof(int) * (size_t)(n > 0 ? n : 1));
        if (end == nullptr) return PADNE_E_NOMEM;
        int *first = row_begin != nullptr ? row_begin : slot_ptr;
        if (n > 0) hipLaunchKernelGGL(slot_row_ends, dim3(nblk(n)), dim3(256), 0, s, n, (const int *)first, row_len, end);
        PADNE_HIP_CHECK(hipGetLastError());
        keep_slots->ctx = ctx;
        keep_slots->n_rows = n;
        keep_slots->n_cols = Y->n_cols;
        keep_slots->n_slots = n_slots;
        keep_slots->begin = first;
        keep_slots->end = end;
        keep_slots->key = key;
        keep_slots->val = val;
        keep_slots->valid = true;
        sc.disown(first);
        sc.disown(key);
        sc.disown(val);
        if (C != nullptr) *C = nullptr;
        return PADNE_OK;
    }
    auto trampoline = [](void *f) -> int { return (*static_cast<const std::function<int()> *>(f))(); };
    return csr_from_slots(ctx, n, Y->n_cols, row_begin != nullptr ? row_begin : slot_ptr, key, val, row_len, C,
                          while_multiplying != nullptr ? +trampoline : nullptr, const_cast<std::function<int()> *>(while_multiplying));
}

__global__ void slot_row_lengths(int n, const int *__restrict__ begin, const int *__restrict__ end, int *__restrict__ len) {
    const int i = blockIdx.x * blockDim.x + threadIdx.x;
    if (i < n) len[i] = end[i] - begin[i];
}

__global__ __launch_bounds__(256) void w_from_slots_kernel(int n, const int *__restrict__ ap_begin,
                                                           const long long *__restrict__ ap_key,
                                                           const double *__restrict__ ap_val, const int *__restrict__ pr,
                                                           const int *__restrict__ pc, const double *__restrict__ pv,
                                                           const double *__restrict__ dinv, const double c,
                                                           const int *__restrict__ wr, int *__restrict__ wc,
                                                           float *__restrict__ wv) {
    __shared__ int rp_all[4][65];
    __shared__ int sp_all[4][65];
    const int lane = threadIdx.x & 63, w = threadIdx.x >> 6;
    int *rp = rp_all[w], *sp = sp_all[w];
    const long long n_wt = ((long long)n + 63) / 64;
    for (long long wt = (long long)blockIdx.x * 4 + w; wt < n_wt; wt += (long long)gridDim.x * 4) {
        const long long r0 = wt * 64;
        const int nr = (int)((n - r0) < 64 ? (n - r0) : 64);
        if (lane <= nr) rp[lane] = wr[r0 + lane];
        if (lane < nr) sp[lane] = ap_begin[r0 + lane];
        if (lane == 0 && nr == 64) rp[64] = wr[r0 + 64];
        asm volatile("s_waitcnt lgkmcnt(0)" ::: "memory");
        __builtin_amdgcn_wave_barrier();
        const int d0 = rp[0], d1 = rp[nr];
        for (int k = d0 + lane; k < d1; k += 64) {
            int lo = 0, hi = nr;
            while (hi - lo > 1) {
                const int mid = (lo + hi) >> 1;
                if (rp[mid] <= k) lo = mid; else hi = mid;
            }
            const int i = (int)r0 + lo;
            const int src = sp[lo] + (k - rp[lo]);
            const int col = (int)(ap_key[src] >> 32);
            double v = -c * dinv[i] * ap_val[src];
            const I2u be = *reinterpret_cast<const I2u *>(pr + i);
            if (be.y - be.x <= 4) {
                const I4u c4 = *reinterpret_cast<const I4u *>(pc + be.x);
                const D2u p0 = *reinterpret_cast<const D2u *>(pv + be.x), p1 = *reinterpret_cast<const D2u *>(pv + be.x + 2);
                const int ln = be.y - be.x;
                if (ln > 0 && c4.x == col) v = p0.x + v;
                if (ln > 1 && c4.y == col) v = p0.y + v;
                if (ln > 2 && c4.z == col) v = p1.x + v;
                if (ln > 3 && c4.w == col) v = p1.y + v;
            } else {
                for (int q = be.x; q < be.y; ++q)
                    if (pc[q] == col) v = pv[q] + v;
            }
            wc[k] = col;
            wv[k] = (float)v;
        }
        if (r0 + nr == n && lane < 4) {
            wc[d1 + lane] = 0;
            wv[d1 + lane] = 0.f;
        }
        asm volatile("" ::: "memory");
        __builtin_amdgcn_wave_barrier();
    }
}

static int build_w_operator(padne_ctx *ctx, const padne_csr *A, const padne_csr *P, const SlotRows &ap, long long n_slots,
                            double c, padne_csr **W_out, int grid_cap = 0, bool with_plan = true) {
    hipStream_t s = ctx->stream;
    const int n = (int)A->n_rows;
    Scratch sc(ctx);
    int *len = nullptr;
    PADNE_TRY(sc.alloc(&len, (size_t)n + 1));
    struct CsrDrop { void operator()(padne_csr *m) const { if (m) padne_csr_destroy(m); } };
    std::unique_ptr<padne_csr, CsrDrop> w_owner(new padne_csr());
    padne_csr *W = w_owner.get();
    W->n_rows = n;
    W->n_cols = P->n_cols;
    W->nnz = n_slots;
    W->device = ctx->device;
    W->owner = ctx;
    W->hierarchy_operator = true;
    W->xw_state = -1;
    W->rowptr = (int32_t *)pool_alloc(ctx, sizeof(int32_t) * ((size_t)n + 1));
    W->cols = (int32_t *)pool_alloc(ctx, sizeof(int32_t) * ((size_t)n_slots + kPadNnz));
    W->vals32 = (float *)pool_alloc(ctx, sizeof(float) * ((size_t)n_slots + kPadNnz));
    if (!W->rowptr || !W->cols || !W->vals32) return PADNE_E_NOMEM;
    hipLaunchKernelGGL(slot_row_lengths, dim3(nblk(n)), dim3(256), 0, s, n, ap.begin, ap.end, len);
    PADNE_HIP_CHECK(hipGetLastError());
    PADNE_TRY(exclusive_scan_i32_async(ctx, len, W->rowptr, n));
    unsigned gw = nblk(((long long)n + 63) / 64, 4);
    if (grid_cap > 0 && gw > (unsigned)grid_cap) gw = (unsigned)grid_cap;
    hipLaunchKernelGGL(w_from_slots_kernel, dim3(gw), dim3(256), 0, s, n, ap.begin, ap.key, ap.val,
                       P->rowptr, P->cols, P->vals, A->dinv, c, (const int *)W->rowptr, W->cols, W->vals32);
    PADNE_HIP_CHECK(hipGetLastError());
    W->xw_state = 0;
    if (with_plan) PADNE_TRY(csr_build_xw_plan_wide(ctx, W, grid_cap));
    if (W->xw_state != 1) W->xw_state = -1;
    *W_out = w_owner.release();
    return PADNE_OK;
}

static int dense_inverse(padne_ctx *ctx, const padne_csr *A, double **inv_out) {
    hipStream_t s = ctx->stream;
    const int n = (int)A->n_rows;
    Scratch sc(ctx);
    double *W = nullptr, *W2 = nullptr, *inv = nullptr;
    PADNE_TRY(sc.alloc(&W, (size_t)n * n));
    PADNE_TRY(sc.alloc(&W2, (size_t)n * n));
    inv = (double *)pool_alloc(ctx, sizeof(double) * (size_t)(n > 0 ? n : 1) * (size_t)(n > 0 ? n : 1));
    if (inv == nullptr) return PADNE_E_NOMEM;
    if (n > 0) {
        hipLaunchKernelGGL(dense_from_csr, dim3(n), dim3(256), 0, s, n, A->rowptr, A->cols, A->vals, W);
        const dim3 ge(nblk(n), (unsigned)((n + kGjStrip - 1) / kGjStrip));
        double *src = W, *dst = W2;
        const bool mfma = !ctx->opt.gj_vector && n > kGjM;
        if (mfma) {
            double *side = nullptr;
            PADNE_TRY(sc.alloc(&side, (size_t)2 * kGjM * kGjM));
            const int n_ct = (n + kGjTC - 1) / kGjTC, n_rt = (n + kGjTR - 1) / kGjTR, n_tiles = n_ct * n_rt;
            const unsigned g64 = 1u + (unsigned)(n_ct * ((n_rt + 3) / 4));
            hipLaunchKernelGGL(gj64_prepare, dim3(1), dim3(256), 0, s, n, 0, std::min(kGjM, n), (const double *)src, side);
            int par = 0;
            for (int k = 0; k < n; k += kGjM) {
                const int bs = std::min(kGjM, n - k);
                const int next_bs = k + kGjM < n ? std::min(kGjM, n - k - kGjM) : 0;
                double *to = k + kGjM >= n ? inv : dst;
                hipLaunchKernelGGL(gj64_step, dim3(g64), dim3(256), 0, s, n, k, bs, (const double *)src, to,
                                   (const double *)(side + (size_t)par * kGjM * kGjM), side + (size_t)(par ^ 1) * kGjM * kGjM,
                                   next_bs, n_ct, n_tiles);
                par ^= 1;
                std::swap(src, dst);
            }
        } else {
            for (int k = 0; k < n; k += kGjBlock) {
                if (n - k >= kGjBlock)
                    hipLaunchKernelGGL(gj_block_step<true>, ge, dim3(256), 0, s, n, k, src, k + kGjBlock >= n ? inv : dst);
                else
                    hipLaunchKernelGGL(gj_block_step<false>, ge, dim3(256), 0, s, n, k, src, inv);
                std::swap(src, dst);
            }
        }
    }
    const hipError_t e = hipGetLastError();
    if (e != hipSuccess) {
        pool_free(ctx, inv);
        set_error("coarse inverse failed: %s", hipGetErrorString(e));
        return PADNE_E_HIP;
    }
    *inv_out = inv;
    return PADNE_OK;
}

void amg_destroy(void *p) {
    Amg *amg = (Amg *)p;
    if (!amg) return;
    (void)hipSetDevice(amg->device);
    for (AmgLevel &L : amg->levels) {
        if (L.A_owned) padne_csr_destroy(L.A_owned);
        if (L.P) padne_csr_destroy(L.P);
        if (L.P_halo) padne_csr_destroy(L.P_halo);
        pool_free(amg->ctx, L.e_ext);
        if (L.R) padne_csr_destroy(L.R);
        if (L.W) padne_csr_destroy(L.W);
        pool_free(amg->ctx, L.b);
        pool_free(amg->ctx, L.xa);
        pool_free(amg->ctx, L.xb);
        pool_free(amg->ctx, L.tmp);
        pool_free(amg->ctx, L.b8);
        pool_free(amg->ctx, L.xa8);
        pool_free(amg->ctx, L.xb8);
// ... 147 lines not shown
        if (lvl > 0 && ((rc = alloc_vec(ctx, &L.b, L.n)) != PADNE_OK || (rc = alloc_vec(ctx, &L.xb, L.n)) != PADNE_OK)) { amg->levels.push_back(L); break; }
        const bool lanczos = lvl > 0 && A->n_rows > ctx->opt.amg_coarse_n;
        bool w_expected = false;
        auto queue_level_extras = [&](const bool ordered = false) -> int {
            if (two && !ordered) PADNE_TRY(stream_order(ctx, aux));
            if (lanczos) {
                Pending *pj = new Pending();
                pj->level = lvl;
                pending.push_back(pj);
                PADNE_TRY(lanczos_enqueue(aux, A, kLanczosSteps, &pj->job));
            }
            if (want_f32) PADNE_TRY(csr_build_f32(aux, const_cast<padne_csr *>(A)));
            if (want_f32 && L.P != nullptr && !w_expected) PADNE_TRY(csr_build_f32(aux, L.P));
            if (want_f32 && L.R != nullptr) PADNE_TRY(csr_build_f32(aux, L.R));
            return PADNE_OK;
        };
        if (coarsest && (rc = queue_level_extras()) != PADNE_OK) { amg->levels.push_back(L); break; }
        if (coarsest) {
            amg->levels.push_back(L);
            break;
        }
        Scratch sc(ctx);
        int *agg = nullptr, n_agg = 0;
        PhaseTimer pt(ctx, amg_verbose());
        double lambda_f = 2.0;
        unsigned char *spos = nullptr;
        int *scol = nullptr;
        float *v32 = nullptr;
        if (want_f32 && A->vals32 == nullptr && A->nnz > 0) {
            padne_csr *Am = const_cast<padne_csr *>(A);
            v32 = (float *)pool_alloc(Am->owner ? Am->owner : ctx, sizeof(float) * ((size_t)A->nnz + kPadNnz));
            if (v32 == nullptr) { rc = PADNE_E_NOMEM; amg->levels.push_back(L); break; }
            Am->vals32 = v32;
        }
        signed char *mis_state = nullptr;
        if ((rc = aggregate(ctx, sc, A, &agg, &n_agg, &lambda_f, &L.lambda, &spos, &scol, v32, &mis_state)) != PADNE_OK) { amg->levels.push_back(L); break; }
        pt.lap("aggregate");
        if (ctx->opt.amg_keep && L.n > 0) {
            L.agg_keep = (int *)pool_alloc(ctx, sizeof(int) * (size_t)L.n);
            L.state_keep = (signed char *)pool_alloc(ctx, (size_t)L.n);
            if (L.agg_keep == nullptr || L.state_keep == nullptr) { rc = PADNE_E_NOMEM; amg->levels.push_back(L); break; }
            hipError_t he = hipMemcpyAsync(L.agg_keep, agg, sizeof(int) * (size_t)L.n, hipMemcpyDeviceToDevice, ctx->stream);
            if (he == hipSuccess) he = hipMemcpyAsync(L.state_keep, mis_state, (size_t)L.n, hipMemcpyDeviceToDevice, ctx->stream);
            if (he != hipSuccess) { set_error("multigrid setup: %s", hipGetErrorString(he)); rc = PADNE_E_HIP; amg->levels.push_back(L); break; }
        }
        if (n_agg == 0 || (double)n_agg > 0.8 * (double)A->n_rows) {
            rc = queue_level_extras();
            amg->levels.push_back(L);
            break;
        }
        if (L.lambda < lambda_f) lambda_f = L.lambda;
        const double omega = kOmegaNum / lambda_f;
        if (amg_verbose())
            fprintf(stderr, "[amg] level %d: n=%lld nnz=%lld lambda=%.3f (P: %.3f) -> %d aggregates\n", lvl,
                    (long long)A->n_rows, (long long)A->nnz, L.lambda, lambda_f, n_agg);
        padne_csr *AP = nullptr, *Ac = nullptr;
        if ((rc = build_prolongator(ctx, A, agg, n_agg, omega, &L.P, spos, scol)) != PADNE_OK) { amg->levels.push_back(L); break; }
        pt.lap("prolongator");
        if (amg_verbose()) fprintf(stderr, "[amg]   P: %lld x %lld nnz=%lld\n", (long long)L.P->n_rows, (long long)L.P->n_cols, (long long)L.P->nnz);
        if (two && (rc = stream_order(ctx, aux)) != PADNE_OK) { amg->levels.push_back(L); break; }
        const std::function<int()> queue_transpose = [&]() -> int { return transpose(aux, L.P, &L.R); };
        SlotRows ap_rows;
        if ((rc = spgemm(ctx, A, L.P, &AP, nullptr, &ap_rows, &queue_transpose)) != PADNE_OK) { amg->levels.push_back(L); break; }
        if (L.R == nullptr && (rc = transpose(aux, L.P, &L.R)) != PADNE_OK) { amg->levels.push_back(L); break; }
        pt.lap("A*P (P^T queued beside it)");
        const bool with_w = lvl == 0 && want_f32 && ap_rows.valid && ctx->opt.amg_w >= 1;
        if (amg_verbose() && AP != nullptr) fprintf(stderr, "[amg]   AP nnz=%lld\n", (long long)AP->nnz);
        if (two && (rc = stream_order(aux, ctx)) != PADNE_OK) { if (AP) padne_csr_destroy(AP); amg->levels.push_back(L); break; }
        if (two && (rc = stream_order(ctx, aux)) != PADNE_OK) { if (AP) padne_csr_destroy(AP); amg->levels.push_back(L); break; }
        w_expected = with_w || (lvl > 0 && want_f32 && w_inner && ap_rows.valid);
        bool side_queued = false;
        const std::function<int()> queue_side = [&]() -> int {
            side_queued = true;
            if (with_w) {
                const double c0 = 1.0 / (0.5 * (L.lambda + L.lambda / kChebRatio));
                PADNE_TRY(build_w_operator(aux, A, L.P, ap_rows, ap_rows.n_slots, c0, &L.W));
            }
            return queue_level_extras(true);
        };
        if (ap_rows.valid) {
            padne_csr ap_shape;
            ap_shape.n_rows = ap_rows.n_rows;
            ap_shape.n_cols = ap_rows.n_cols;
            rc = spgemm(ctx, L.R, &ap_shape, &Ac, &ap_rows, nullptr, nullptr, &queue_side);
        } else {
            rc = spgemm(ctx, L.R, AP, &Ac, nullptr, nullptr, nullptr, &queue_side);
        }
        if (rc == PADNE_OK && !side_queued) rc = queue_side();
        if (rc != PADNE_OK && two) (void)hipStreamSynchronize(aux->stream);
        pt.lap("R*(AP)");
        if (amg_verbose() && rc == PADNE_OK) fprintf(stderr, "[amg]   Ac: n=%lld nnz=%lld\n", (long long)Ac->n_rows, (long long)Ac->nnz);
        if (AP) padne_csr_destroy(AP);
        auto take_slots = [](SlotRows &to, SlotRows &from) {
            std::swap(to.ctx, from.ctx);
            std::swap(to.begin, from.begin);
            std::swap(to.end, from.end);
            std::swap(to.key, from.key);
            std::swap(to.val, from.val);
            to.n_rows = from.n_rows;
            to.n_cols = from.n_cols;
            to.n_slots = from.n_slots;
            to.valid = from.valid;
        };
        if (with_w) {
            take_slots(ap_keep, ap_rows);
        } else if (lvl > 0 && rc == PADNE_OK && want_f32 && w_inner && ap_rows.valid) {
            ap_inner.emplace_back(new KeptSlots());
            ap_inner.back()->level = lvl;
            take_slots(ap_inner.back()->rows, ap_rows);
        }
        ap_rows.release();
        amg->levels.push_back(L);
        if (rc != PADNE_OK) break;
        if ((rc = csr_build_dinv(ctx, Ac)) != PADNE_OK) { padne_csr_destroy(Ac); break; }
        Ac->hierarchy_operator = true;
        amg->levels.back().P->hierarchy_operator = true;
        amg->levels.back().R->hierarchy_operator = true;
        A = Ac;
    }
    if (rc == PADNE_OK) {
        const AmgLevel &last = amg->levels.back();
        if (last.P != nullptr) {
            rc = PADNE_E_NOCOARSEN;
            set_error("multigrid setup did not reach a coarsest level");
        } else if (last.n > 4096) {
            rc = PADNE_E_NOCOARSEN;
            set_error("multigrid coarsening stalled at %lld unknowns", last.n);
        } else {
            amg->n_coarse = (int)last.n;
            PhaseTimer pd(ctx, amg_verbose());
            if (two && !ap_inner.empty()) rc = stream_order(ctx, aux);
            if (rc == PADNE_OK) rc = dense_inverse(ctx, last.A, &amg->coarse_inv);
            pd.lap("dense inverse");
        }
    }
    if (rc != PADNE_OK) {
        drop_pending();
        if (two) (void)hipStreamSynchronize(aux->stream);
        amg_destroy(amg);
        return rc;
    }
    for (Pending *pj : pending) {
        double ritz = 0.0;
        const int rcl = lanczos_finish(&pj->job, &ritz);
        if (rcl != PADNE_OK && rc == PADNE_OK) rc = rcl;
        AmgLevel &L = amg->levels[(size_t)pj->level];
        const double est = 1.08 * ritz;
        if (rcl == PADNE_OK && est > 0.0 && est < L.lambda) L.lambda = est;
        delete pj;
    }
    pending.clear();
    for (AmgLevel &L : amg->levels) L.jac = 1.0 / (0.5 * (L.lambda + L.lambda / kChebRatio));
    for (auto &ks : ap_inner) {
        if (rc != PADNE_OK) break;
        AmgLevel &L = amg->levels[(size_t)ks->level];
        if (L.P == nullptr || L.A->dinv == nullptr) continue;
        rc = build_w_operator(aux, L.A, L.P, ks->rows, ks->rows.n_slots, L.jac, &L.W, 512, false);
    }
    for (AmgLevel &L : amg->levels)
        if (rc == PADNE_OK && want_f32 && L.P != nullptr && L.W == nullptr) rc = csr_build_f32(aux, L.P);
    if (rc == PADNE_OK && two) rc = stream_order(aux, ctx);
    if (rc != PADNE_OK) {
        if (two) (void)hipStreamSynchronize(aux->stream);
        amg_destroy(amg);
        return rc;
    }
    amg->operator_complexity = nnz_total / (double)(A0->nnz > 0 ? A0->nnz : 1);
    if (want_f32 && amg->levels.size() >= 2) {
        hipStream_t s = ctx->stream;
        if (amg->levels[0].b == nullptr && (rc = alloc_vec(ctx, &amg->levels[0].b, amg->levels[0].n)) != PADNE_OK) {
            amg_destroy(amg);
            return rc;
        }
        if (amg->n_coarse > 0) {
            const size_t cnt = (size_t)amg->n_coarse * (size_t)amg->n_coarse;
            amg->coarse_inv32 = (float *)pool_alloc(ctx, sizeof(float) * cnt);
            if (amg->coarse_inv32 == nullptr) {
                amg_destroy(amg);
                return PADNE_E_NOMEM;
// ... 407 lines not shown
        for (int q = 0; q < W; ++q) {
            n_glob += (long long)sts[(size_t)q * 2];
            n_max = std::max(n_max, (long long)sts[(size_t)q * 2]);
            lam = std::max(lam, sts[(size_t)q * 2 + 1]);
        }
        Lr.lambda = lam;
        const bool coarsest = lvl > 0 && (n_glob <= gather_n || lvl == kMaxLevels - 1);
        if (lvl > 0 && !coarsest) {
            double ritz = 0.0;
            if ((rc = estimate_lambda_max(ctx, A, kLanczosSteps, &ritz, &plan)) != PADNE_OK) break;
            const double est = 1.08 * ritz;
            if (est > 0.0 && est < Lr.lambda) Lr.lambda = est;
        }
        Lr.jac = 1.0 / (0.5 * (Lr.lambda + Lr.lambda / kChebRatio));
        if ((rc = alloc_vec(ctx, &Lr.xa, Lr.n + (long long)W * plan.m)) != PADNE_OK) break;
        if ((rc = alloc_vec(ctx, &Lr.tmp, A->n_rows)) != PADNE_OK) break;
        if (lvl > 0 && ((rc = alloc_vec(ctx, &Lr.b, Lr.n)) != PADNE_OK ||
                        (rc = alloc_vec(ctx, &Lr.xb, Lr.n + (long long)W * plan.m)) != PADNE_OK)) break;
        if (lvl > 0 && (rc = hipMemsetAsync(Lr.xb, 0, sizeof(double) * (size_t)(Lr.n + (long long)W * plan.m), s) == hipSuccess
                                 ? PADNE_OK : PADNE_E_HIP) != PADNE_OK) break;
        if ((rc = hipMemsetAsync(Lr.xa, 0, sizeof(double) * (size_t)(Lr.n + (long long)W * plan.m), s) == hipSuccess
                      ? PADNE_OK : PADNE_E_HIP) != PADNE_OK) break;
        if (coarsest) break;
        PhaseTimer pt(ctx, amg_verbose() && ctx->rank == 0);
        padne_csr *blk = nullptr;
        if ((rc = owned_block(ctx, A, Lr.n, &blk)) != PADNE_OK) break;
        Scratch sc(ctx);
        int *agg = nullptr, n_agg = 0;
        double lambda_f = 2.0, lambda_g = 2.0;
        signed char *mis_state = nullptr;
        if ((rc = csr_build_dinv(ctx, blk)) == PADNE_OK &&
            (rc = aggregate(ctx, sc, blk, &agg, &n_agg, &lambda_f, nullptr, nullptr, nullptr, nullptr, &mis_state)) == PADNE_OK)
            rc = gershgorin(ctx, blk, &lambda_g, false);
        if (rc == PADNE_OK && ctx->opt.amg_keep && Lr.n > 0) {
            Lr.agg_keep = (int *)pool_alloc(ctx, sizeof(int) * (size_t)Lr.n);
            Lr.state_keep = (signed char *)pool_alloc(ctx, (size_t)Lr.n);
            if (Lr.agg_keep == nullptr || Lr.state_keep == nullptr) rc = PADNE_E_NOMEM;
            hipError_t he = rc == PADNE_OK ? hipMemcpyAsync(Lr.agg_keep, agg, sizeof(int) * (size_t)Lr.n, hipMemcpyDeviceToDevice, s)
                                           : hipSuccess;
            if (rc == PADNE_OK && he == hipSuccess)
                he = hipMemcpyAsync(Lr.state_keep, mis_state, (size_t)Lr.n, hipMemcpyDeviceToDevice, s);
            if (he != hipSuccess) { set_error("multigrid setup: %s", hipGetErrorString(he)); rc = PADNE_E_HIP; }
        }
        if (rc != PADNE_OK) { padne_csr_destroy(blk); break; }
        std::vector<double> ag = {(double)n_agg}, ags;
        if ((rc = host_allgather(ctx, ag, ags)) != PADNE_OK) { padne_csr_destroy(blk); break; }
        long long agg_glob = 0;
        for (int q = 0; q < W; ++q) agg_glob += (long long)ags[(size_t)q];
        if (amg_verbose() && ctx->rank == 0)
            fprintf(stderr, "[amg] level %d: global n=%lld (this rank %lld, nnz %lld, m=%d) lambda=%.3f -> %lld aggregates\n",
                    lvl, n_glob, Lr.n, (long long)A->nnz, plan.m, Lr.lambda, agg_glob);
        if (agg_glob == 0 || (double)agg_glob > 0.8 * (double)n_glob) {
            padne_csr_destroy(blk);
            stalled = true;
            if (lvl == 0) {
                rc = PADNE_E_NOCOARSEN;
                set_error("row-partitioned multigrid: no coarsening on the finest level");
            }
            break;
        }
        if (lambda_g < lambda_f) lambda_f = lambda_g;
        pt.lap("block+aggregate");
        rc = build_prolongator(ctx, blk, agg, n_agg, kOmegaNum / lambda_f, &Lr.P);
        padne_csr_destroy(blk);
        if (rc != PADNE_OK) break;
        if ((rc = transpose(ctx, Lr.P, &Lr.R)) != PADNE_OK) break;
        pt.lap("prolongator+transpose");
        padne_csr *P_halo = nullptr, *P_ext = nullptr, *AP = nullptr, *Ac = nullptr;
        std::vector<int> export_c;
        int m_c = 0;
        if ((rc = exchange_prolongator_rows(ctx, Lr, Lr.P, n_agg, export_c, &m_c, &P_halo)) != PADNE_OK) break;
        rc = csr_vstack(ctx, Lr.P, P_halo, (long long)n_agg + (long long)W * m_c, &P_ext);
        P_halo->hierarchy_operator = true;
        Lr.P_halo = P_halo;
        if (rc != PADNE_OK) break;
        pt.lap("exchange P rows");
        SlotRows ap_rows;
        rc = spgemm(ctx, A, P_ext, &AP, nullptr, &ap_rows);
        if (rc != PADNE_OK) { padne_csr_destroy(P_ext); break; }
        if (ap_rows.valid) {
            padne_csr ap_shape;
            ap_shape.n_rows = ap_rows.n_rows;
            ap_shape.n_cols = ap_rows.n_cols;
            rc = spgemm(ctx, Lr.R, &ap_shape, &Ac, &ap_rows);
            if (rc == PADNE_OK && want_f32 && A->dinv != nullptr && (ctx->opt.amg_w == 2 || (ctx->opt.amg_w == 1 && lvl == 0))) {
                rc = build_w_operator(ctx, A, Lr.P, ap_rows, ap_rows.n_slots, Lr.jac, &Lr.W, 0, lvl == 0);
                if (rc == PADNE_OK) Lr.W->n_cols = P_ext->n_cols;
            }
        } else {
            rc = spgemm(ctx, Lr.R, AP, &Ac);
        }
        ap_rows.release();
        padne_csr_destroy(P_ext);
        if (AP) padne_csr_destroy(AP);
        if (rc != PADNE_OK) break;
        if ((rc = csr_build_dinv(ctx, Ac)) != PADNE_OK) { padne_csr_destroy(Ac); break; }
        pt.lap("galerkin");
        Ac->hierarchy_operator = true;
        Lr.P->hierarchy_operator = true;
        Lr.R->hierarchy_operator = true;
        export_owned = (int32_t *)pool_alloc(ctx, sizeof(int32_t) * (export_c.empty() ? 1 : export_c.size()));
        if (export_owned == nullptr) { padne_csr_destroy(Ac); rc = PADNE_E_NOMEM; break; }
        if (!export_c.empty()) {
            hipError_t e = hipMemcpyAsync(export_owned, export_c.data(), sizeof(int) * export_c.size(),
                                          hipMemcpyHostToDevice, s);
            if (e == hipSuccess) e = hipStreamSynchronize(s);
            if (e != hipSuccess) { padne_csr_destroy(Ac); pool_free(ctx, export_owned); export_owned = nullptr; rc = PADNE_E_HIP; break; }
        }
        plan.n_owned = n_agg;
        plan.m = m_c;
        plan.n_export = (int)export_c.size();
        plan.export_idx = export_owned;
        export_host = export_c;
        A = Ac;
    }
    if (export_owned != nullptr) pool_free(ctx, export_owned);
    if (rc == PADNE_OK) {
        if (amg->levels.back().P != nullptr && !stalled) {
            rc = PADNE_E_NOCOARSEN;
            set_error("multigrid setup did not reach a coarsest level");
        } else {
            PhaseTimer pg(ctx, amg_verbose() && ctx->rank == 0);
            rc = gather_tail(ctx, amg);
            pg.lap("gather + tail hierarchy");
        }
    }
    if (rc != PADNE_OK) {
        amg_destroy(amg);
        return rc;
    }
    amg->operator_complexity = nnz_total / (double)(A0->nnz > 0 ? A0->nnz : 1);
    if ((rc = enable_f32(ctx, amg, want_f32 ? 1 : 0)) != PADNE_OK) {
        amg_destroy(amg);
        return rc;
    }
    PADNE_HIP_CHECK(hipStreamSynchronize(s));
    amg->setup_seconds = std::chrono::duration<double>(std::chrono::steady_clock::now() - t_begin).count();
    A0->amg = amg;
    return PADNE_OK;
}

int amg_apply(padne_ctx *ctx, const padne_csr *A0, const double *r, double *z, double *partials_rz,
              const int32_t *done_flag, const double *bb2, bool entry_done, float *z32 = nullptr);

static int amg_apply_f32(padne_ctx *ctx, Amg *amg, const double *r, double *z, double *partials_rz,
                         const int32_t *done_flag, const double *bb2, bool entry_done, float *z32) {
    hipStream_t s = ctx->stream;
    const int nl = (int)amg->levels.size();
    if (partials_rz == nullptr) {
        set_error("the single-precision cycle is only used as the CG preconditioner");
        return PADNE_E_INVALID;
    }
    bool fused_start = false;
    auto exit_stage = [&](const padne_csr *m, int mode, const float *x, ProductArgs<float> a, int part) {
        a.dot_with = r;
        a.partials = partials_rz;
        a.out_scale2 = bb2;
        return z32 != nullptr ? launch_spmv<float, float>(ctx, m, mode, x, z32, a, part)
                              : launch_spmv<float, double>(ctx, m, mode, x, z, a, part);
    };
    const bool local_halo = amg->dist && nl >= 2 && amg->levels[nl - 2].P_halo != nullptr &&
                            amg->levels[nl - 2].P_halo->vals32 != nullptr && amg->levels[nl - 2].e_ext != nullptr &&
                            amg->tail_slot_idx != nullptr;
    for (int l = 0; l < nl; ++l) {
        AmgLevel &L = amg->levels[l];
        float *b = (float *)L.b, *xa = (float *)L.xa, *tmp = (float *)L.tmp;
        if (l == nl - 1) {
            if (amg->dist) {
                float *cg = (float *)amg->coarse_gather;
                float *seg = cg + (size_t)ctx->rank * amg->n_pad;
                PADNE_HIP_CHECK(hipMemcpyAsync(seg, b, sizeof(float) * (size_t)L.n, hipMemcpyDeviceToDevice, s));
                PADNE_TRY(comm_allgather_f32(ctx, seg, cg, amg->n_pad));
                hipLaunchKernelGGL(compact_pieces<float>, dim3(nblk(amg->n_pad), ctx->world), dim3(256), 0, s, ctx->world,
// ... 391 lines not shown
```

### padne_amd/csrc/assemble.hip

```cpp
#include "common.hpp"
#include "face.hpp"

#include <atomic>

#include <cmath>

#include <algorithm>

#include <string.h>

namespace padne {

constexpr int kScanItems = 16;
constexpr int kScanChunk = 256 * kScanItems;

__device__ __forceinline__ int block_exclusive_scan_256(int v, int *lds , int *total) {
    const int lane = threadIdx.x & 63, w = threadIdx.x >> 6;
    int inc = v;
#pragma unroll
    for (int off = 1; off < 64; off <<= 1) {
        const int t = __shfl_up(inc, off, 64);
        if (lane >= off) inc += t;
    }
    if (lane == 63) lds[w] = inc;
// ... 1382 lines not shown
            bool keep = false;
            int c = 0;
            double v = 0.0;
            if (e < n) {
                c = (int)(ks[e] >> 32);
                const bool head = e == 0 || (int)(ks[e - 1] >> 32) != c;
                if (head) {
                    int i = e;
                    while (i < n && (int)(ks[i] >> 32) == c && (unsigned)(ks[i] & 0xffffffffLL) < 2u) ++i;
                    if (mesh_row) {
                        if (c == r) v = sig * dacc;
                        else if (i > e) v = sig * gm[e];
                    }
                    while (i < n && (int)(ks[i] >> 32) == c) {
                        v = v + vs[i];
                        ++i;
                    }
                    keep = v != 0.0;
                }
            }
            const unsigned long long mk = __ballot(keep);
            if (keep) {
                const int o = base + __popcll(mk & ((1ull << lane) - 1ull));
                key[s0 + o] = (long long)c << 32;
                val[s0 + o] = v;
            }
            base += __popcll(mk);
        }
        if (lane == 0) row_len[r] = base;
        asm volatile("s_waitcnt vmcnt(0) lgkmcnt(0)" ::: "memory");
        __builtin_amdgcn_wave_barrier();
    }
}

template <int CAP>
__global__ __launch_bounds__(128) void merge_rows_lds(long long n_rows, const int *__restrict__ slot_ptr,
                                                      long long *__restrict__ key, double *__restrict__ val,
                                                      int *__restrict__ row_len) {
    __shared__ long long Kc[CAP][128];
    __shared__ double Vc[CAP][128];
    const int t = threadIdx.x;
    const long long r = (long long)blockIdx.x * 128 + t;
    if (r >= n_rows) return;
    const int s0 = slot_ptr[r];
    const int n = slot_ptr[r + 1] - s0;
    if (n > CAP) return;
    for (int i = 0; i < n; ++i) {
        const long long k = key[s0 + i];
        const double v = val[s0 + i];
        int j = i - 1;
        while (j >= 0 && Kc[j][t] > k) {
            Kc[j + 1][t] = Kc[j][t];
            Vc[j + 1][t] = Vc[j][t];
            --j;
        }
        Kc[j + 1][t] = k;
        Vc[j + 1][t] = v;
    }
    int o = 0, i = 0;
    while (i < n) {
        const int col = (int)(Kc[i][t] >> 32);
        double v = 0.0;
        while (i < n && (int)(Kc[i][t] >> 32) == col) {
            v = v + Vc[i][t];
            ++i;
        }
        if (v != 0.0) {
            key[s0 + o] = (long long)col << 32;
            val[s0 + o] = v;
            ++o;
        }
    }
    row_len[r] = o;
}

static int compact_rows_per_wave(long long n_rows, long long nnz) {
    if (n_rows <= 0 || n_rows > 100000 || nnz <= 16 * n_rows) return 64;
    return nnz <= 128 * n_rows ? 8 : 1;
}

__global__ __launch_bounds__(256) void compact_rows(long long n_rows, const int *__restrict__ slot_ptr,
                                                    const int *__restrict__ rowptr, const long long *__restrict__ key,
                                                    const double *__restrict__ val, int *__restrict__ cols,
                                                    double *__restrict__ vals, const int rpw) {
    __shared__ int rp_all[4][65];
    __shared__ int sp_all[4][65];
    const int lane = threadIdx.x & 63, w = threadIdx.x >> 6;
    int *rp = rp_all[w], *sp = sp_all[w];
    const long long n_wt = (n_rows + rpw - 1) / rpw;
    for (long long wt = (long long)blockIdx.x * 4 + w; wt < n_wt; wt += (long long)gridDim.x * 4) {
        const long long r0 = wt * rpw;
        const int nr = (int)((n_rows - r0) < rpw ? (n_rows - r0) : rpw);
        if (lane <= nr) rp[lane] = rowptr[r0 + lane];
        if (lane < nr) sp[lane] = slot_ptr[r0 + lane];
        if (lane == 0 && nr == 64) rp[64] = rowptr[r0 + 64];
        asm volatile("s_waitcnt lgkmcnt(0)" ::: "memory");
        __builtin_amdgcn_wave_barrier();
        const int d0 = rp[0], d1 = rp[nr];
        for (int k = d0 + lane; k < d1; k += 64) {
            int lo = 0, hi = nr;
            while (hi - lo > 1) {
                const int mid = (lo + hi) >> 1;
                if (rp[mid] <= k) lo = mid; else hi = mid;
            }
            const int src = sp[lo] + (k - rp[lo]);
            cols[k] = (int)(key[src] >> 32);
            vals[k] = val[src];
        }
        asm volatile("" ::: "memory");
        __builtin_amdgcn_wave_barrier();
    }
}

__global__ void fill_value_i32(int *p, long long n, int v) {
    const long long i = (long long)blockIdx.x * blockDim.x + threadIdx.x;
    if (i < n) p[i] = v;
}

__global__ void reduce_count(long long n_rows, const int *__restrict__ rowptr, const int *__restrict__ cols,
                             const int *__restrict__ map, const int *__restrict__ cmap, int *__restrict__ cnt) {
    const long long r = (long long)blockIdx.x * blockDim.x + threadIdx.x;
    if (r >= n_rows) return;
    const int t = map[r];
    if (t < 0) return;
    int c = 0;
    for (int k = rowptr[r]; k < rowptr[r + 1]; ++k) c += (cmap[cols[k]] >= 0) ? 1 : 0;
    if (c) atomicAdd(&cnt[t], c);
}

__global__ void reduce_fill(long long n_rows, const int *__restrict__ rowptr, const int *__restrict__ cols,
                            const double *__restrict__ vals, const int *__restrict__ map,
                            const int *__restrict__ cmap, double scale,
                            const int *__restrict__ slot_ptr, int *__restrict__ cursor,
                            long long *__restrict__ key, double *__restrict__ val) {
    const long long r = (long long)blockIdx.x * blockDim.x + threadIdx.x;
    if (r >= n_rows) return;
    const int t = map[r];
    if (t < 0) return;
    int c = 0;
    for (int k = rowptr[r]; k < rowptr[r + 1]; ++k) c += (cmap[cols[k]] >= 0) ? 1 : 0;
    if (!c) return;
    int s = slot_ptr[t] + atomicAdd(&cursor[t], c);
    for (int k = rowptr[r]; k < rowptr[r + 1]; ++k) {
        const int tc = cmap[cols[k]];
        if (tc < 0) continue;
        key[s] = make_key(tc, k);
        val[s] = scale * vals[k];
        ++s;
    }
}


__global__ void map_is_injective(long long n, const int *__restrict__ map, int n_out, int *__restrict__ hist,
                                 int *__restrict__ flag) {
    const long long i = (long long)blockIdx.x * blockDim.x + threadIdx.x;
    if (i >= n) return;
    const int t = map[i];
    if (t < -1 || t >= n_out) {
        *(volatile int *)(flag + 1) = 1;
        return;
    }
    if (t >= 0 && atomicAdd(&hist[t], 1) > 0) *(volatile int *)flag = 1;
}

__global__ void relabel_count_direct(long long n_rows, const int *__restrict__ rowptr, const int *__restrict__ cols,
                                     const int *__restrict__ map, const int *__restrict__ cmap, int *__restrict__ cnt) {
    const long long r = (long long)blockIdx.x * blockDim.x + threadIdx.x;
    if (r >= n_rows) return;
    const int t = map[r];
    if (t < 0) return;
    int c = 0;
    for (int k = rowptr[r]; k < rowptr[r + 1]; ++k) c += (cmap[cols[k]] >= 0) ? 1 : 0;
    cnt[t] = c;
}

template <int CAP>
__global__ __launch_bounds__(128) void relabel_fill_direct(long long n_rows, const int *__restrict__ rowptr,
                                                           const int *__restrict__ cols, const double *__restrict__ vals,
                                                           const int *__restrict__ map, const int *__restrict__ cmap,
                                                           double scale, const int *__restrict__ out_rowptr,
                                                           int *__restrict__ out_cols, double *__restrict__ out_vals,
                                                           int *__restrict__ zero_seen) {
    __shared__ int Cc[CAP][128];
    __shared__ double Vc[CAP][128];
    const int th = threadIdx.x;
    const long long r = (long long)blockIdx.x * 128 + th;
    if (r >= n_rows) return;
    const int t = map[r];
    if (t < 0) return;
    const int o0 = out_rowptr[t], n_out = out_rowptr[t + 1] - o0;
// ... 267 lines not shown
                if (keep) {
                    const int pos = o + __popcll(b & lt);
                    const double wv = scale * v[j];
                    zero = zero || wv == 0.0;
                    out_cols[pos] = tc[j];
                    out_vals[pos] = wv;
                }
                o += __popcll(b);
            }
        }
    }
    if (zero) *(volatile int *)zero_seen = 1;
}

static thread_local bool t_partial_mesh = false;
static std::atomic<long long> g_two_pass_fallbacks{0};

static int merge_listed_mesh_rows(padne_ctx *ctx, long long n_vert, int n_mesh, const long long *d_voff, const double *d_sigma,
                                  const int *slot_ptr, long long *key, double *val, int *row_len, int *d_err,
                                  const int *row_list, const int *n_list_dev, long long n_merge) {
    hipStream_t s = ctx->stream;
    if (n_merge <= 0) return PADNE_OK;
    hipLaunchKernelGGL(merge_rows_mesh_wave, dim3(std::min(nblk(n_merge, 4), 8192u)), dim3(256), 0, s, n_list_dev, row_list,
                       n_vert, n_mesh, d_voff, d_sigma, slot_ptr, key, val, row_len, d_err);
    PADNE_HIP_CHECK(hipGetLastError());
    int h_long[ERR_WORDS];
    PADNE_TRY(read_back(ctx, d_err, sizeof(h_long), h_long));
    if (h_long[ERR_LONG_ROWS]) {
        hipLaunchKernelGGL((sort_long_rows_wave<kWaveSortCap, 4>), dim3(std::min(nblk(n_merge, 16), 8192u)), dim3(256), 0, s,
                           n_merge, row_list, slot_ptr, key, val, kMergeWaveCap + 1, 1);
        hipLaunchKernelGGL(merge_rows<true>, dim3(nblk(n_merge, 128)), dim3(128), 0, s, n_merge, n_vert, n_mesh, d_voff,
                           d_sigma, slot_ptr, key, val, row_len, d_err, kMergeWaveCap + 1, row_list, kWaveSortCap);
        PADNE_HIP_CHECK(hipGetLastError());
    }
    return PADNE_OK;
}

static int finish_rows(padne_ctx *ctx, Scratch &sc, long long n_rows, long long n_cols, const int *slot_ptr, long long *key,
                       double *val, padne_csr **out) {
    hipStream_t s = ctx->stream;
    int *row_len = nullptr;
    PADNE_TRY(sc.alloc(&row_len, (size_t)n_rows + 1));
    PADNE_TRY(merge_slots_generic(ctx, n_rows, slot_ptr, key, val, row_len));
    int *rowptr_tmp = nullptr;
    PADNE_TRY(sc.alloc(&rowptr_tmp, (size_t)n_rows + 1));
    int64_t nnz = 0;
    PADNE_TRY(exclusive_scan_i32(ctx, row_len, rowptr_tmp, n_rows, &nnz));
    padne_csr *m = nullptr;
    PADNE_TRY(csr_alloc(ctx, n_rows, n_cols, nnz, &m));
    hipError_t e = hipMemcpyAsync(m->rowptr, rowptr_tmp, sizeof(int32_t) * (size_t)(n_rows + 1),
                                  hipMemcpyDeviceToDevice, s);
    if (e == hipSuccess) {
        const int rpw = compact_rows_per_wave(n_rows, nnz);
        hipLaunchKernelGGL(compact_rows, dim3(std::min(nblk((n_rows + rpw - 1) / rpw, 4), 65536u)), dim3(256), 0, s, n_rows, slot_ptr,
                           m->rowptr, key, val, m->cols, m->vals, rpw);
        e = hipGetLastError();
    }
    if (e == hipSuccess) e = hipStreamSynchronize(s);
    if (e != hipSuccess) {
        set_error("row compaction failed: %s", hipGetErrorString(e));
        padne_csr_destroy(m);
        return PADNE_E_HIP;
    }
    *out = m;
    return PADNE_OK;
}


int merge_slots_generic(padne_ctx *ctx, long long n_rows, const int *slot_ptr, long long *key, double *val,
                        int *row_len) {
    constexpr int kLdsCap = 32;
    hipLaunchKernelGGL(merge_rows_lds<kLdsCap>, dim3(nblk(n_rows, 128)), dim3(128), 0, ctx->stream, n_rows, slot_ptr, key,
                       val, row_len);
    hipLaunchKernelGGL(sort_long_rows_wave<kWaveSortCap>, dim3(std::min(nblk(n_rows, 256), 2048u)), dim3(256), 0, ctx->stream,
                       n_rows, (const int *)nullptr, slot_ptr, key, val, kLdsCap + 1, 0);
    hipLaunchKernelGGL(merge_rows<false>, dim3(nblk(n_rows, 128)), dim3(128), 0, ctx->stream, n_rows, 0LL, 0,
                       (const long long *)nullptr, (const double *)nullptr, slot_ptr, key, val, row_len,
                       (int *)nullptr, kLdsCap + 1, (const int *)nullptr, kWaveSortCap);
    PADNE_HIP_CHECK(hipGetLastError());
    return PADNE_OK;
}

int csr_from_slots(padne_ctx *ctx, long long n_rows, long long n_cols, const int *slot_ptr, const long long *key,
                   const double *val, const int *row_len, padne_csr **out, int (*while_scanning)(void *), void *while_scanning_arg) {
    hipStream_t s = ctx->stream;
    Scratch sc(ctx);
    int *rowptr_tmp = nullptr;
    PADNE_TRY(sc.alloc(&rowptr_tmp, (size_t)n_rows + 1));
    int64_t nnz = 0;
    {
        ScanTicket ticket;
        long long h[2] = {0, 0};
        PADNE_TRY(scan_i32_begin(ctx, row_len, rowptr_tmp, n_rows, &ticket, true));
        const int rc_cb = while_scanning != nullptr ? while_scanning(while_scanning_arg) : PADNE_OK;
        const int rc_scan = scan_i32_end(ctx, &ticket, h);
        PADNE_TRY(rc_cb);
        PADNE_TRY(rc_scan);
        if (h[0] < 0 || h[1] != 0) {
            set_error("scan of negative counts");
            return PADNE_E_INVALID;
        }
        if (h[0] >= 2147483647LL) {
            set_error("%lld entries exceed the 32-bit index space", h[0]);
            return PADNE_E_TOOLARGE;
        }
        nnz = h[0];
    }
    padne_csr *m = nullptr;
    PADNE_TRY(csr_alloc(ctx, n_rows, n_cols, nnz, &m));
    hipError_t e = hipMemcpyAsync(m->rowptr, rowptr_tmp, sizeof(int32_t) * (size_t)(n_rows + 1),
                                  hipMemcpyDeviceToDevice, s);
    if (e == hipSuccess && n_rows > 0) {
        const int rpw = compact_rows_per_wave(n_rows, nnz);
        hipLaunchKernelGGL(compact_rows, dim3(std::min(nblk((n_rows + rpw - 1) / rpw, 4), 65536u)), dim3(256), 0, s, n_rows, slot_ptr,
                           m->rowptr, key, val, m->cols, m->vals, rpw);
        e = hipGetLastError();
    }
    if (e != hipSuccess) {
        set_error("row compaction failed: %s", hipGetErrorString(e));
        padne_csr_destroy(m);
        return PADNE_E_HIP;
    }
    *out = m;
    return PADNE_OK;
}

__global__ void unpack_slots_kernel(long long nnz, const long long *__restrict__ key, const double *__restrict__ val,
                                    int *__restrict__ cols, double *__restrict__ vals) {
    for (long long k = (long long)blockIdx.x * blockDim.x + threadIdx.x; k < nnz; k += (long long)gridDim.x * blockDim.x) {
        cols[k] = (int)(key[k] >> 32);
        vals[k] = val[k];
    }
}

int sort_slots_exact(padne_ctx *ctx, long long n_rows, const int *slot_ptr, long long *key, double *val, int *row_len_scratch) {
    Scratch sc(ctx);
    int *long_list = nullptr;
    PADNE_TRY(sc.alloc(&long_list, (size_t)n_rows + 1));
    int *n_long = row_len_scratch + n_rows;
    PADNE_HIP_CHECK(hipMemsetAsync(n_long, 0, sizeof(int), ctx->stream));
    hipLaunchKernelGGL((sort_long_rows_wave<64, 8>), dim3(std::min(nblk(n_rows, 32), 8192u)), dim3(256), 0, ctx->stream, n_rows,
                       (const int *)nullptr, slot_ptr, key, val, 2, 0, n_long, (const int *)nullptr, long_list);
    hipLaunchKernelGGL(sort_listed_rows_block, dim3(1024), dim3(256), 0, ctx->stream, (const int *)n_long, (const int *)long_list,
                       slot_ptr, key, val);
    hipLaunchKernelGGL(merge_rows<false>, dim3(nblk(n_rows, 128)), dim3(128), 0, ctx->stream, n_rows, 0LL, 0,
                       (const long long *)nullptr, (const double *)nullptr, slot_ptr, key, val, row_len_scratch,
                       (int *)nullptr, kWaveSortCap + 1);
    PADNE_HIP_CHECK(hipGetLastError());
    return PADNE_OK;
}

int csr_from_exact_slots(padne_ctx *ctx, long long n_rows, long long n_cols, long long nnz, const int *slot_ptr,
                         const long long *key, const double *val, padne_csr **out) {
    hipStream_t s = ctx->stream;
    padne_csr *m = nullptr;
    PADNE_TRY(csr_alloc(ctx, n_rows, n_cols, nnz, &m));
    hipError_t e = hipMemcpyAsync(m->rowptr, slot_ptr, sizeof(int32_t) * (size_t)(n_rows + 1), hipMemcpyDeviceToDevice, s);
    if (e == hipSuccess && nnz > 0) {
        hipLaunchKernelGGL(unpack_slots_kernel, dim3((unsigned)std::min<long long>((nnz + 255) / 256, 8192)), dim3(256), 0, s,
                           nnz, key, val, m->cols, m->vals);
        e = hipGetLastError();
    }
    if (e != hipSuccess) {
        set_error("slot unpacking failed: %s", hipGetErrorString(e));
        padne_csr_destroy(m);
        return PADNE_E_HIP;
    }
    *out = m;
    return PADNE_OK;
}

}

using namespace padne;

extern "C" int padne_assemble_system_ex(padne_ctx *ctx, int64_t n_unknowns, int64_t n_vert, const double *xy_host,
                                        int64_t n_tri, const int32_t *tri_host, int64_t n_mesh,
                                        const int64_t *mesh_vertex_offset, const int64_t *mesh_tri_offset,
                                        const double *conductance, int64_t n_coo, const int64_t *coo_row,
                                        const int64_t *coo_col, const double *coo_val, int32_t flags, padne_csr **out) {
    struct Guard {
        ~Guard() { t_partial_mesh = false; }
    } guard;
    t_partial_mesh = (flags & 1) != 0;
    return padne_assemble_system(ctx, n_unknowns, n_vert, xy_host, n_tri, tri_host, n_mesh, mesh_vertex_offset,
                                 mesh_tri_offset, conductance, n_coo, coo_row, coo_col, coo_val, out);
}

extern "C" int padne_assemble_system(padne_ctx *ctx, int64_t n_unknowns, int64_t n_vert, const double *xy_host,
                                     int64_t n_tri, const int32_t *tri_host, int64_t n_mesh,
                                     const int64_t *mesh_vertex_offset, const int64_t *mesh_tri_offset,
                                     const double *conductance, int64_t n_coo, const int64_t *coo_row,
                                     const int64_t *coo_col, const double *coo_val, padne_csr **out) {
    PADNE_REQUIRE(ctx && out, "null argument");
    PADNE_REQUIRE(n_unknowns >= 0 && n_vert >= 0 && n_tri >= 0 && n_mesh >= 0 && n_coo >= 0, "negative size");
    PADNE_REQUIRE(n_vert <= n_unknowns, "more vertices than unknowns");
    PADNE_REQUIRE(n_unknowns < 2147483647LL, "too many unknowns for int32 indices");
    PADNE_REQUIRE(n_vert == 0 || xy_host, "xy");
// ... 651 lines not shown
```

### padne_amd/csrc/capi.hip

```cpp
#include "common.hpp"

#include <algorithm>

#include <math.h>
#include <stdarg.h>
#include <string.h>
#include <chrono>

namespace padne {

std::atomic<long long> g_launch_count{0};

void options_from_env(padne_options *o) {
    *o = padne_options();
    auto on = [](const char *name) { const char *e = getenv(name); return e != nullptr && e[0] != '\0' && !(e[0] == '0' && e[1] == '\0'); };
    auto has = [](const char *list, const char *word) {
        const size_t n = strlen(word);
        for (const char *p = list; p != nullptr && *p != '\0';) {
            const char *q = strchr(p, ',');
            const size_t len = q != nullptr ? (size_t)(q - p) : strlen(p);
            if (len >= n && strncmp(p, word, n) == 0 && (len == n || p[n] == ':')) return p;
            p = q != nullptr ? q + 1 : nullptr;
        }
        return (const char *)nullptr;
    };
    o->amg_f64 = on("PADNE_AMG_F64");
    if (const char *e = getenv("PADNE_AMG_W")) o->amg_w = strcmp(e, "none") == 0 ? 0 : (strcmp(e, "fine") == 0 ? 1 : 2);
    o->amg_exchange_all = on("PADNE_AMG_EXCHANGE_ALL");
    o->amg_keep = on("PADNE_AMG_KEEP");
    o->pcg_p64 = on("PADNE_PCG_P64");
    o->pcg_no_xhist = on("PADNE_PCG_NO_XHIST");
    o->gj_vector = on("PADNE_GJ_VECTOR");
    o->no_batch = on("PADNE_NO_BATCH");
    o->no_mailbox = on("PADNE_NO_MAILBOX");
    o->no_p2p = on("PADNE_NO_P2P");
    o->no_split = on("PADNE_NO_SPLIT");
    o->no_xwindow = on("PADNE_NO_XWINDOW");
    o->setup_one_stream = on("PADNE_SETUP_ONE_STREAM");
    if (const char *e = getenv("PADNE_CG_SINGLE_REDUCTION")) o->cg_single_reduction = atoi(e) != 0 ? 1 : 0;
    if (const char *e = getenv("PADNE_LOCKSTEP_NARROW")) o->lockstep_narrow = atoi(e);
    if (const char *e = getenv("PADNE_AMG_COARSE_N")) o->amg_coarse_n = std::min(4096, std::max(16, atoi(e)));
    if (const char *e = getenv("PADNE_AMG_GATHER_N")) o->amg_gather_n = atoll(e);
    if (const char *e = getenv("PADNE_P2P_TIMEOUT_MS")) {
        const long v = atol(e);
        if (v > 0 && v <= 600000) o->p2p_timeout_ms = (unsigned)v;
    }
    if (const char *f = getenv("PADNE_FORCE")) {
        o->force_asm_hash = has(f, "asm_hash") != nullptr;
        o->force_asm_two_pass = has(f, "asm_two_pass") != nullptr;
        o->force_relabel_slots = has(f, "relabel_slots") != nullptr;
        o->force_transpose_cursors = has(f, "transpose_cursors") != nullptr;
        o->force_xhist_small = has(f, "xhist_small") != nullptr;
        o->force_relabel_lanes = has(f, "relabel_lanes") != nullptr;
        if (const char *w = has(f, "spgemm_split")) o->force_spgemm_split = w[12] == ':' ? atoll(w + 13) : 30000;
    }
    if (const char *e = getenv("PADNE_POOL_GUARD")) {
        char *end = nullptr;
        const long v = strtol(e, &end, 16);
        if (end != e && *end == '\0' && strlen(e) <= 2 && v >= 0 && v <= 255) o->pool_guard = (int)v;
    }
    if (const char *v = getenv("PADNE_VERBOSE")) {
        o->verbose_amg = has(v, "amg") != nullptr;
        o->verbose_xw = has(v, "xw") != nullptr;
        o->verbose_pool = has(v, "pool") != nullptr;
    }
}

static thread_local char g_err[1024] = "";

void set_error(const char *fmt, ...) {
    va_list ap;
    va_start(ap, fmt);
    vsnprintf(g_err, sizeof(g_err), fmt, ap);
    va_end(ap);
}

static int workspace_poison(padne_ctx *ctx) {
    PADNE_HIP_CHECK(hipMemsetAsync(ctx->ws, ctx->opt.pool_guard, ctx->ws_bytes, ctx->stream));
    PADNE_HIP_CHECK(hipStreamSynchronize(ctx->stream));
    return PADNE_OK;
}

int ensure_workspace(padne_ctx *ctx, size_t bytes) {
    if (ctx->ws_bytes >= bytes) return ctx->opt.pool_guard < 0 ? PADNE_OK : workspace_poison(ctx);
    if (ctx->ws) {
        PADNE_HIP_CHECK(hipStreamSynchronize(ctx->stream));
        PADNE_HIP_CHECK(hipFree(ctx->ws));
        ctx->ws = nullptr;
        ctx->ws_bytes = 0;
    }
    if (hipMalloc(&ctx->ws, bytes) != hipSuccess) {
        set_error("hipMalloc of %zu workspace bytes failed", bytes);
        return PADNE_E_NOMEM;
    }
    ctx->ws_bytes = bytes;
    return ctx->opt.pool_guard < 0 ? PADNE_OK : workspace_poison(ctx);
}

constexpr size_t kPoolCacheLimit = (size_t)240 << 30;

static unsigned char pool_canary(const padne_ctx *ctx) { return ctx->opt.pool_guard == 0xa5 ? 0xc3 : 0xa5; }

static int pool_guard_arm(padne_ctx *ctx, void *p) {
    const PoolBook::Block &b = *ctx->pool.find(p);
    char *base = (char *)b.base;
    PADNE_HIP_CHECK(hipMemsetAsync(base, b.canary, b.front(), ctx->stream));
    if (b.requested > 0) PADNE_HIP_CHECK(hipMemsetAsync(p, ctx->opt.pool_guard, b.requested, ctx->stream));
    PADNE_HIP_CHECK(hipMemsetAsync(base + b.back_begin(), b.canary, b.back_bytes(), ctx->stream));
    PADNE_HIP_CHECK(hipStreamSynchronize(ctx->stream));
    ++ctx->pool_guard_allocs;
    return PADNE_OK;
}

static void pool_guard_check(padne_ctx *ctx, const PoolBook::Block &b) {
    if (hipDeviceSynchronize() != hipSuccess) {
        (void)hipGetLastError();
        return;
    }
    std::vector<unsigned char> h(std::max(b.front(), b.back_bytes()));
    for (int side = 1; side <= 2; ++side) {
        const size_t begin = side == 1 ? 0 : b.back_begin(), len = side == 1 ? b.front() : b.back_bytes();
        if (hipMemcpy(h.data(), (const char *)b.base + begin, len, hipMemcpyDeviceToHost) != hipSuccess) {
            (void)hipGetLastError();
            return;
        }
        size_t i = 0;
        while (i < len && h[i] == b.canary) ++i;
        if (i == len) continue;
        padne_ctx::PoolViolation v;
        v.requested = (long long)b.requested;
        v.side = side;
        v.offset = (long long)(begin + i) - (long long)b.front();
        if (ctx->pool_guard_violations++ == 0) ctx->pool_first_violation = v;
        ctx->pool_last_violation = v;
        set_error("pool guard: a block of %lld bytes was written %s: first changed byte at offset %lld of the block",
                  v.requested, side == 1 ? "in front of its start" : "behind its end", v.offset);
// ... 602 lines not shown
```

### padne_amd/csrc/common.hpp

```cpp
#pragma once

#include <hip/hip_runtime.h>
#include <stdint.h>
#include <stdio.h>
#include <map>
#include <string>
#include <unordered_map>
#include <vector>

#include "../../include/padne_hip.h"
#include "../../include/padne_hip_test.h"
#include "../../include/padne_hip_probe.h"
#include "pool_book.hpp"

#include <atomic>

namespace padne {

extern std::atomic<long long> g_launch_count;

void set_error(const char *fmt, ...);

#define PADNE_HIP_CHECK(expr)                                                              \
    do {                                                                                   \
// ... 15 lines not shown

#define PADNE_TRY(...)                                                                     \
    do {                                                                                   \
        int _rc = (__VA_ARGS__);                                                           \
        if (_rc != PADNE_OK) return _rc;                                                   \
    } while (0)

}
#undef hipLaunchKernelGGL
#define hipLaunchKernelGGL(kernelName, numBlocks, numThreads, memPerBlock, streamId, ...)   \
    do {                                                                                   \
        ::padne::g_launch_count.fetch_add(1, std::memory_order_relaxed);                   \
        kernelName<<<(numBlocks), (numThreads), (memPerBlock), (streamId)>>>(__VA_ARGS__); \
    } while (0)
#define hipMemsetAsync(...) (::padne::g_launch_count.fetch_add(1, std::memory_order_relaxed), hipMemsetAsync(__VA_ARGS__))
namespace padne {

constexpr int kNumXcd = 8;

constexpr int kSpmvThreads = 256;
constexpr int kSpmvRows = 256;
constexpr int kPadNnz = 4096;

constexpr int kMaxPartials = 2048;
constexpr int kPinnedSlots = 16;
constexpr int kPinnedSlotBase = 4096;
constexpr int kPinnedBytes = kPinnedSlotBase + 512 * kPinnedSlots;

constexpr int kTinySystem = 32;
constexpr int kSpmmK = 8;

}

struct padne_csr {
    int64_t n_rows = 0, n_cols = 0, nnz = 0;
    int32_t *rowptr = nullptr;
    int32_t *cols = nullptr;
    double *vals = nullptr;
    double *dinv = nullptr;
    int device = 0;
    padne_ctx *owner = nullptr;
    void *amg = nullptr;
    float *vals32 = nullptr, *dinv32 = nullptr;
    int4 *xw_desc = nullptr;
    unsigned short *xw_lidx = nullptr;
    int xw_state = 0;
    int xw_run = 0;
    int xw_nruns = 3;
    int *split_tiles = nullptr;
    int split_n_int = 0, split_n_bnd = 0;
    int split_state = 0;
    bool hierarchy_operator = false;
    bool cols_unsorted = false;
    padne_csr *prec_block = nullptr;
    double *mesh_xy = nullptr, *mesh_sigma = nullptr;
    int32_t *mesh_tri = nullptr;
    long long *mesh_voff = nullptr, *mesh_toff = nullptr;
    int64_t mesh_n_vert = 0, mesh_n_tri = 0, mesh_n_mesh = 0;
};

struct padne_options {
    bool amg_f64 = false;
    int amg_w = 2;
    bool amg_exchange_all = false;
    bool pcg_p64 = false;
    bool pcg_no_xhist = false;
    bool gj_vector = false;
    bool no_batch = false;
    bool no_mailbox = false;
    bool no_p2p = false;
    bool no_split = false;
    bool no_xwindow = false;
    bool amg_keep = false;
    bool setup_one_stream = false;
    int cg_single_reduction = -1;
    int lockstep_narrow = -1;
    int amg_coarse_n = 2048;
    long long amg_gather_n = 0;
    unsigned p2p_timeout_ms = 20000;
    bool force_asm_hash = false, force_asm_two_pass = false, force_relabel_slots = false, force_transpose_cursors = false;
    bool force_relabel_lanes = false;
    bool force_xhist_small = false;
    long long force_spgemm_split = 0;
    bool verbose_amg = false, verbose_xw = false, verbose_pool = false;
    int pool_guard = -1;
};
namespace padne { void options_from_env(padne_options *o); }

struct padne_ctx {
    int device = 0;
    padne_options opt;
    hipStream_t stream = nullptr;
    double *partials = nullptr;
    double *scalars = nullptr;
    int32_t *status = nullptr;
    void *pinned = nullptr;
    void *ws = nullptr;
    size_t ws_bytes = 0;
    void *comm = nullptr;
    void *team = nullptr;
    int rank = 0, world = 1;
    bool halo_on = false;
    long long halo_n_owned = 0;
    int halo_m = 0, halo_n_export = 0;
    int32_t *halo_export = nullptr;
    void *p2p_mbox = nullptr;
    void **p2p_peers = nullptr;
    int p2p_m_cap = 0;
    unsigned long long p2p_seq = 0;
    bool p2p_ipc = false;
    std::vector<void *> p2p_ipc_mapped;
    unsigned p2p_timeout_ms = 20000;
    int (*hostcoll_fn)(void *, const void *, void *, int64_t) = nullptr;
    void *hostcoll_user = nullptr;
    hipEvent_t ev0 = nullptr, ev1 = nullptr;
    hipStream_t copy_stream[4] = {nullptr, nullptr, nullptr, nullptr};
    padne_ctx *aux = nullptr, *parent = nullptr;
    bool is_aux = false;
    unsigned long long lockstep_groups = 0;
    unsigned pinned_busy = 0;
    unsigned long long *mailbox = nullptr, *mailbox_dev = nullptr;
    unsigned long long mail_seq = 0;
    hipEvent_t ev_order = nullptr;
    padne::PoolBook pool;
    struct PoolViolation { long long requested = 0, side = 0, offset = 0; };
    long long pool_guard_allocs = 0, pool_guard_violations = 0;
    PoolViolation pool_first_violation, pool_last_violation;
};

namespace padne {

int ensure_workspace(padne_ctx *ctx, size_t bytes);
int csr_alloc(padne_ctx *ctx, int64_t n_rows, int64_t n_cols, int64_t nnz, padne_csr **out);
int csr_shrink_nnz(padne_ctx *ctx, padne_csr *m, int64_t nnz);
int csr_build_dinv(padne_ctx *ctx, padne_csr *m);

int spmv_grid(const padne_csr *m);
enum { SPMV_PLAIN = 0, SPMV_DOT = 1, SPMV_RESID = 2, SPMV_ADD = 3, SPMV_JACOBI = 4,
       SPMV_DOT_AUX = 5,
       SPMV_WUP = 6,
       SPMV_RESTRICT = 7,
       SPMV_RESID_PRE = 8 };
enum { SPMV_ALL = 0, SPMV_INTERIOR = 1, SPMV_BOUNDARY = 2 };

template <typename XT> struct ProductArgs {
    const XT *b = nullptr;
    const XT *dinv = nullptr;
    XT scale = 0;
    const XT *x_pre = nullptr;
    XT *y2 = nullptr;
    const XT *rhs = nullptr;
    const double *dot_with = nullptr;
    double *partials = nullptr;
    const double *out_scale2 = nullptr;
    const int32_t *done_flag = nullptr;
};
template <typename XT> inline const XT *product_vals(const padne_csr *m) {
    if constexpr (sizeof(XT) == 4) return m->vals32;
    else return m->vals;
}

template <typename XT, typename YT, typename ST = XT>
int launch_spmv(padne_ctx *ctx, const padne_csr *m, int mode, const ST *x, YT *y, const ProductArgs<XT> &a, int part = SPMV_ALL);
template <typename XT, typename YT>
int launch_spmm(padne_ctx *ctx, const padne_csr *m, int k, int mode, const XT *x, YT *y, const ProductArgs<XT> &a);
inline int launch_spmv(padne_ctx *ctx, const padne_csr *m, const double *x, double *y, const double *dot_with, double *partials,
// ... 51 lines not shown
int comm_p2p_check(padne_ctx *ctx);
bool comm_exchange_overlaps(const padne_ctx *ctx);
int comm_p2p_begin(padne_ctx *ctx, int m, void ***peers_dev, size_t *entry_offset);
int comm_p2p_arrive(padne_ctx *ctx);
void comm_p2p_release(padne_ctx *ctx);

struct HaloPlan {
    long long n_owned = 0;
    int m = 0, n_export = 0;
    const int32_t *export_idx = nullptr;
};
int halo_exchange_plan(padne_ctx *ctx, const HaloPlan &plan, double *v, const int32_t *done_flag);
int halo_exchange_plan_f32(padne_ctx *ctx, const HaloPlan &plan, float *v, const int32_t *done_flag);
struct HaloTicket {
    bool p2p = false;
    size_t entry_off = 0;
    unsigned long long seq1 = 0;
};
int halo_send(padne_ctx *ctx, const HaloPlan &plan, double *v, const int32_t *done_flag, HaloTicket *tk);
int halo_send_f32(padne_ctx *ctx, const HaloPlan &plan, float *v, const int32_t *done_flag, HaloTicket *tk);
int halo_recv(padne_ctx *ctx, const HaloPlan &plan, double *v, const int32_t *done_flag, const HaloTicket &tk);
int halo_recv_f32(padne_ctx *ctx, const HaloPlan &plan, float *v, const int32_t *done_flag, const HaloTicket &tk);

void amg_destroy(void *amg);
int estimate_lambda_max(padne_ctx *ctx, const padne_csr *a, int steps, double *lambda, const HaloPlan *plan = nullptr);
struct LanczosJob {
    padne_ctx *ctx = nullptr;
    int steps = 0;
    double *hist = nullptr;
    std::vector<double> host;
    double *host_dst = nullptr;
    int pinned_slot = -1;
};
int lanczos_enqueue(padne_ctx *ctx, const padne_csr *a, int steps, LanczosJob *job, const HaloPlan *plan = nullptr);
int lanczos_finish(LanczosJob *job, double *lambda);
int csr_vstack(padne_ctx *ctx, const padne_csr *top, const padne_csr *bottom, int64_t n_cols, padne_csr **out);
int launch_power_density_block(padne_ctx *ctx, const padne_csr *m, int n_cols, const double *V_dev, double *out_dev,
                               int *bad_dev);
int launch_sensitivity_block(padne_ctx *ctx, const padne_csr *m, const long long *tile_off_host, int n_cols, int n_obj,
                             const double *W_dev, const double *V_dev, double *power_dev, double *density_dev, double *total_dev,
                             int *bad_dev);
int launch_current_faces(padne_ctx *ctx, const padne_csr *m, const long long *tile_dev, long long n_blocks, int n_cols,
                         int n_report, const double *V_dev, double *J_dev, double *mag_dev, double *env_dev, int *env_case_dev,
                         double *box_dev, double *mesh_max_dev, long long *mesh_face_dev, double *mesh_power_dev, int *bad_dev);
int launch_current_cuts(padne_ctx *ctx, const padne_csr *m, const long long *tile_dev, int n_cols, int n_report,
                        const double *V_dev, int n_cut, const double *cut_xy_dev, long long n_pairs, const int *pair_cut_dev,
                        const long long *pair_tile_dev, const long long *pair_off_host, double *cut_dev, int *bad_dev);
int launch_combine_block(padne_ctx *ctx, long long N, int n_cols, int n_out, long long nnz, const int *w_ptr_dev,
                         const int *w_col_dev, const double *w_val_dev, const double *V_dev, double *out_dev);

void *pool_alloc(padne_ctx *ctx, size_t bytes);
void pool_free(padne_ctx *ctx, void *p);
void pool_release_all(padne_ctx *ctx);

struct Scratch {
    padne_ctx *ctx;
    std::vector<void *> ptrs;
    explicit Scratch(padne_ctx *c) : ctx(c) {}
    ~Scratch() { release(); }
    void release() {
        for (void *p : ptrs) if (p) pool_free(ctx, p);
        ptrs.clear();
    }
    void disown(void *p) {
        for (void *&q : ptrs) if (q == p) q = nullptr;
    }
    template <typename T> int alloc(T **out, size_t count) {
        void *p = pool_alloc(ctx, sizeof(T) * (count ? count : 1));
        if (p == nullptr) return PADNE_E_NOMEM;
        ptrs.push_back(p);
        *out = (T *)p;
        return PADNE_OK;
    }
};
static inline unsigned nblk(long long n, int bs = 256) {
    const long long b = (n + bs - 1) / bs;
    return (unsigned)(b > 0 ? b : 1);
}
int merge_slots_generic(padne_ctx *ctx, long long n_rows, const int *slot_ptr, long long *key, double *val,
                        int *row_len);
int sort_slots_exact(padne_ctx *ctx, long long n_rows, const int *slot_ptr, long long *key, double *val, int *row_len_scratch);
int csr_from_slots(padne_ctx *ctx, long long n_rows, long long n_cols, const int *slot_ptr, const long long *key,
                   const double *val, const int *row_len, padne_csr **out,
                   int (*while_scanning)(void *) = nullptr, void *while_scanning_arg = nullptr);
int csr_from_exact_slots(padne_ctx *ctx, long long n_rows, long long n_cols, long long nnz, const int *slot_ptr,
                         const long long *key, const double *val, padne_csr **out);

}
```

Before: 32.45 solves/s.

## Fold AMG setup passes into producer kernels (MIS round, dinv, row ends, redo flag)

Folds several standalone AMG setup kernels into their producers. strength_mark now computes the first neighbour-max priority round. compact_rows computes dinv/dinv32 for the coarse operator. The SpGEMM kernels write row end offsets and lists of overflowed rows directly, and the prolongator kernel sets the redo flag itself. This is meant to cut kernel launches and extra passes over the matrices during setup, at the cost of LDS atomics and more register pressure in hot setup kernels. It only affects setup time, so the effect on solves/s depends on whether setup is counted in the measurement.

```diff
diff --git a/padne_amd/csrc/amg.hip b/padne_amd/csrc/amg.hip
--- a/padne_amd/csrc/amg.hip
+++ b/padne_amd/csrc/amg.hip
@@ -133,14 +133,17 @@
                                                      const int4 *__restrict__ xw_desc = nullptr,
                                                      const unsigned char *__restrict__ xw_lidx = nullptr,
                                                      const int xw_run = 0, unsigned char *__restrict__ spos = nullptr,
-                                                     float *__restrict__ vals32 = nullptr) {
+                                                     float *__restrict__ vals32 = nullptr,
+                                                     unsigned int *__restrict__ m1 = nullptr) {
     constexpr int CH = 512;
     __shared__ unsigned char rid_all[4 * CH];
     __shared__ double pv_all[4 * CH];
     __shared__ double red[4], red2[4];
+    __shared__ unsigned int top_all[4 * 64];
     const int lane = threadIdx.x & 63, w = threadIdx.x >> 6;
     unsigned char *rid = rid_all + w * CH;
     double *pv = pv_all + w * CH;
+    unsigned int *top = top_all + w * 64;
     const XcdSweep sw = xcd_sweep(n_wtiles, 4, w);
     double my_max = 0.0, my_plain = 0.0;
     for (long long wt = sw.t0; wt < sw.t1; wt += sw.stride) {
@@ -161,6 +164,7 @@
         if (spos != nullptr) dsc = xw_desc[wt];
         const bool windowed = spos != nullptr && dsc.w != 0;
         const int self_pos = windowed ? xw_position(dsc, xw_run, r) : 0;
+        if (m1 != nullptr) top[lane] = prio32_of(r);
         for (int base = k0; base < k1; base += CH) {
             const int lo = max(rs, base), hi = min(re, base + CH);
             for (int k = lo; k < hi; ++k) rid[k - base] = (unsigned char)lane;
@@ -180,6 +184,7 @@
                     const bool st = c != i && strong(v, dr, dinv[c], theta2);
                     scol[e] = st ? c : i;
                     if (windowed) spos[e] = st ? xw_lidx[e] : (unsigned char)sp;
+                    if (m1 != nullptr && st) atomicMax(&top[rl], prio32_of(c));
                     if (bound_partial != nullptr) {
                         rid[e - base] = (unsigned char)(rl | (c == i ? 0x40 : 0) | (st ? 0x80 : 0));
                         pv[e - base] = v;
@@ -200,6 +205,13 @@
                 }
             }
             asm volatile("" ::: "memory");
+            __builtin_amdgcn_wave_barrier();
+        }
+        if (m1 != nullptr) {
+            asm volatile("s_waitcnt lgkmcnt(0)" ::: "memory");
+            __builtin_amdgcn_wave_barrier();
+            if (r < row1) m1[r] = top[lane];
+            asm volatile("s_waitcnt lgkmcnt(0)" ::: "memory");
             __builtin_amdgcn_wave_barrier();
         }
         if (bound_partial != nullptr && r < row1) {
@@ -1080,7 +1092,8 @@
 __global__ void spgemm_rows(int n_rows, const int *__restrict__ xr, const int *__restrict__ xc,
                             const double *__restrict__ xv, const int *__restrict__ yr, const int *__restrict__ yc,
                             const double *__restrict__ yv, const int *__restrict__ ye, const int ycs, const int *__restrict__ slot_ptr,
-                            long long *__restrict__ key, double *__restrict__ val, int *__restrict__ row_len) {
+                            long long *__restrict__ key, double *__restrict__ val, int *__restrict__ row_len,
+                            int *__restrict__ row_end = nullptr) {
     const int i = blockIdx.x * blockDim.x + threadIdx.x;
     if (i >= n_rows) return;
     long long *K = key + slot_ptr[i];
@@ -1111,6 +1124,7 @@
         }
     }
     row_len[i] = m;
+    if (row_end != nullptr) row_end[i] = slot_ptr[i] + m;
 }
 
 template <int CAP, int KC, int QC, int YCS>
@@ -1119,7 +1133,9 @@
                                                             const int *__restrict__ yc, const double *__restrict__ yv,
                                                             const int *__restrict__ ye, const int *__restrict__ slot_ptr,
                                                             long long *__restrict__ key, double *__restrict__ val,
-                                                            int *__restrict__ row_len, int *__restrict__ begin) {
+                                                            int *__restrict__ row_len, int *__restrict__ begin,
+                                                            int *__restrict__ row_end, int *__restrict__ pend,
+                                                            int *__restrict__ pend_count) {
     static_assert(CAP % 2 == 0, "keys are kept in pairs");
     __shared__ int2 Kc[CAP / 2][128];
     __shared__ double Vc[CAP][128];
@@ -1225,8 +1241,10 @@
     if (!live) return;
     if (overflow) {
         row_len[i] = -1;
+        if (pend != nullptr) pend[atomicAdd(pend_count, 1)] = i;
         return;
     }
+    if (row_end != nullptr) row_end[i] = place + m;
     long long *K = key + place;
     double *V = val + place;
     int kr[CAP];
@@ -1398,7 +1416,8 @@
                                                          const int *__restrict__ slot_ptr, long long *__restrict__ key,
                                                          double *__restrict__ val, int *__restrict__ row_len,
                                                          const int *__restrict__ row_list = nullptr,
-                                                         const int *__restrict__ list_count = nullptr) {
+                                                         const int *__restrict__ list_count = nullptr,
+                                                         int *__restrict__ row_end = nullptr) {
     constexpr int G = 256 / LANES;
     __shared__ SpgemmRowLds<CAPP, HT, LANES> s_rows[G];
     const int lane = threadIdx.x & 63;
@@ -1461,7 +1480,10 @@
         advance();
         const int nd = spgemm_row_by_masks<CAPP, HT, LANES>(s_rows[g], sl, sub, has_row, nx, len, ystart, a, yc, yv, ycs,
                                                             key + place, val + place);
-        if (has_row && sl == 0) row_len[i] = nd;
+        if (has_row && sl == 0) {
+            row_len[i] = nd;
+            if (nd >= 0 && row_end != nullptr) row_end[i] = place + nd;
+        }
     }
 }
 
@@ -1471,7 +1493,8 @@
                                                          const int *__restrict__ slot_ptr, long long *__restrict__ key,
                                                          double *__restrict__ val, int *__restrict__ row_len,
                                                          const int only_pending, const int *__restrict__ row_list = nullptr,
-                                                         const int *__restrict__ list_count = nullptr) {
+                                                         const int *__restrict__ list_count = nullptr,
+                                                         int *__restrict__ row_end = nullptr) {
     extern __shared__ double acc_and_flag[];
     double *acc = acc_and_flag;
     unsigned char *hit = (unsigned char *)(acc + n_cols);
@@ -1517,7 +1540,10 @@
         base += total;
         __syncthreads();
     }
-    if (threadIdx.x == 0) row_len[i] = base;
+    if (threadIdx.x == 0) {
+        row_len[i] = base;
+        if (row_end != nullptr) row_end[i] = slot_ptr[i] + base;
+    }
     }
 }
 
@@ -1543,7 +1569,8 @@
 __global__ void spgemm_rows_redo(int n_rows, const int *__restrict__ xr, const int *__restrict__ xc,
                                  const double *__restrict__ xv, const int *__restrict__ yr, const int *__restrict__ yc,
                                  const double *__restrict__ yv, const int *__restrict__ ye, const int ycs, const int *__restrict__ slot_ptr,
-                                 long long *__restrict__ key, double *__restrict__ val, int *__restrict__ row_len) {
+                                 long long *__restrict__ key, double *__restrict__ val, int *__restrict__ row_len,
+                                 int *__restrict__ row_end = nullptr) {
     const int i = blockIdx.x * blockDim.x + threadIdx.x;
     if (i >= n_rows || row_len[i] >= 0) return;
     long long *K = key + slot_ptr[i];
@@ -1574,6 +1601,7 @@
         }
     }
     row_len[i] = m;
+    if (row_end != nullptr) row_end[i] = slot_ptr[i] + m;
 }
 
 __global__ void dense_from_csr(int n, const int *__restrict__ rowptr, const int *__restrict__ cols,
@@ -2098,6 +2126,7 @@
                      float *vals32_out = nullptr, signed char **state_out = nullptr) {
     hipStream_t s = ctx->stream;
     const int n = (int)A->n_rows;
+    const bool folded = !(ctx->opt.force_amg_unfolded & 1);
     const double theta2 = kTheta * kTheta;
     signed char *state = nullptr;
     unsigned int *w0 = nullptr, *w1 = nullptr, *w2 = nullptr;
@@ -2133,23 +2162,25 @@
                        spos != nullptr ? spos + A->nnz : (unsigned char *)nullptr, kPadNnz);
     hipLaunchKernelGGL(strength_mark, gm, b, 0, s, n, n_wt, A->rowptr, A->cols, A->vals, A->dinv, theta2, scol, bound_part,
                        xw ? A->xw_desc : (const int4 *)nullptr, xw ? (const unsigned char *)A->xw_lidx : (const unsigned char *)nullptr,
-                       xw ? A->xw_run : 0, spos, vals32_out);
+                       xw ? A->xw_run : 0, spos, vals32_out, folded ? w1 : (unsigned int *)nullptr);
     PADNE_HIP_CHECK(hipGetLastError());
     const bool long_rows = !xw && n <= 65536 && A->nnz >= 24LL * n;
-    auto launch_round = [&](int *open_counter) {
+    auto launch_round = [&](int *open_counter, const bool have_m1) {
         if (xw) {
-            hipLaunchKernelGGL((nbr_max_xw<unsigned int, false>), gm, b, 0, s, n, n_wt, srow, scol, spos, A->xw_desc, A->xw_run,
-                               (const unsigned int *)w0, w1, (unsigned int *)nullptr, (signed char *)nullptr, (int *)nullptr);
+            if (!have_m1)
+                hipLaunchKernelGGL((nbr_max_xw<unsigned int, false>), gm, b, 0, s, n, n_wt, srow, scol, spos, A->xw_desc, A->xw_run,
+                                   (const unsigned int *)w0, w1, (unsigned int *)nullptr, (signed char *)nullptr, (int *)nullptr);
             hipLaunchKernelGGL((nbr_max_xw<unsigned int, true>), gm, b, 0, s, n, n_wt, srow, scol, spos, A->xw_desc, A->xw_run,
                                (const unsigned int *)w1, (unsigned int *)nullptr, w0, state, open_counter);
         } else if (long_rows) {
-            hipLaunchKernelGGL(nbr_max_wpr<unsigned int>, dim3((unsigned)((n + 3) / 4)), b, 0, s, n, srow, (const int *)scol,
-                               (const unsigned int *)w0, w1);
+            if (!have_m1)
+                hipLaunchKernelGGL(nbr_max_wpr<unsigned int>, dim3((unsigned)((n + 3) / 4)), b, 0, s, n, srow, (const int *)scol,
+                                   (const unsigned int *)w0, w1);
             hipLaunchKernelGGL(nbr_max_wpr<unsigned int>, dim3((unsigned)((n + 3) / 4)), b, 0, s, n, srow, (const int *)scol,
                                (const unsigned int *)w1, w2);
             hipLaunchKernelGGL(mis_decide, dim3(std::min<unsigned>(g.x, 1024u)), b, 0, s, n, w0, w2, state, open_counter);
         } else {
-            hipLaunchKernelGGL(nbr_max<unsigned int>, gm, b, 0, s, n, n_wt, srow, scol, w0, w1);
+            if (!have_m1) hipLaunchKernelGGL(nbr_max<unsigned int>, gm, b, 0, s, n, n_wt, srow, scol, w0, w1);
             hipLaunchKernelGGL(nbr_max<unsigned int>, gm, b, 0, s, n, n_wt, srow, scol, w1, w2);
             hipLaunchKernelGGL(mis_decide, dim3(std::min<unsigned>(g.x, 1024u)), b, 0, s, n, w0, w2, state, open_counter);
         }
@@ -2171,7 +2202,7 @@
     while (round < kMaxRounds && open_count > 0 && (!compact_ok || round < 2 || open_count > n / 8)) {
         const int reps = (round == 0 && compact_ok && full_batch < 2) ? 2 : full_batch;
         for (int rep = 0; rep < reps && round < kMaxRounds; ++rep, ++round) {
-            launch_round(counter + round);
+            launch_round(counter + round, folded && round == 0);
         }
         PADNE_HIP_CHECK(hipGetLastError());
         PADNE_TRY(count_back(counter + round - 1, &open_count));
@@ -2247,7 +2278,8 @@
                                                         const double *__restrict__ vals, const double *__restrict__ dinv,
                                                         double theta2, double omega, const int *__restrict__ agg,
                                                         const int *__restrict__ slot_ptr, long long *__restrict__ key,
-                                                        double *__restrict__ val, int *__restrict__ row_len) {
+                                                        double *__restrict__ val, int *__restrict__ row_len,
+                                                        int *__restrict__ any) {
     static_assert(CAP % 2 == 0, "keys are kept in pairs");
     __shared__ int2 Kc[CAP / 2][128];
     __shared__ double Vc[CAP][128];
@@ -2328,6 +2360,7 @@
     }
     if (overflow) {
         row_len[i] = -1;
+        if (any != nullptr) atomicOr(any, 1);
         return;
     }
     int o = 0;
@@ -2525,6 +2558,7 @@
                              padne_csr **P, const unsigned char *spos = nullptr, const int *scol = nullptr) {
     hipStream_t s = ctx->stream;
     const int n = (int)A->n_rows;
+    const bool folded = !(ctx->opt.force_amg_unfolded & 16);
     Scratch sc(ctx);
     if (spos != nullptr && scol != nullptr && A->xw_state == 1 && A->xw_run <= 85 && n > 0 &&
         (long long)A->nnz + (long long)n < 2147483647LL) {
@@ -2565,8 +2599,8 @@
     PADNE_HIP_CHECK(hipMemsetAsync(any, 0, sizeof(int), s));
     hipLaunchKernelGGL(prolong_slot_ptr, dim3(nblk((long long)n + 1)), dim3(256), 0, s, n, A->rowptr, slot_ptr);
     hipLaunchKernelGGL(prolong_rows_lds<24>, dim3(nblk(n, 128)), dim3(128), 0, s, n, A->rowptr, A->cols, A->vals, A->dinv,
-                       kTheta * kTheta, omega, agg, slot_ptr, key, val, row_len);
-    hipLaunchKernelGGL(prolong_redo_flag, dim3(nblk(n)), dim3(256), 0, s, n, row_len, any);
+                       kTheta * kTheta, omega, agg, slot_ptr, key, val, row_len, folded ? any : (int *)nullptr);
+    if (!folded) hipLaunchKernelGGL(prolong_redo_flag, dim3(nblk(n)), dim3(256), 0, s, n, row_len, any);
     PADNE_HIP_CHECK(hipGetLastError());
     int h_any = 0;
     PADNE_TRY(read_back(ctx, any, sizeof(int), &h_any));
@@ -2627,6 +2661,7 @@
     padne_ctx *ctx = nullptr;
     long long n_rows = 0, n_cols = 0, n_slots = 0;
     int *begin = nullptr, *end = nullptr;
+    int *len = nullptr;
     long long *key = nullptr;
     double *val = nullptr;
     bool valid = false;
@@ -2635,10 +2670,11 @@
         if (ctx != nullptr) {
             pool_free(ctx, begin);
             pool_free(ctx, end);
+            pool_free(ctx, len);
             pool_free(ctx, key);
             pool_free(ctx, val);
         }
-        begin = end = nullptr;
+        begin = end = len = nullptr;
         key = nullptr;
         val = nullptr;
         valid = false;
@@ -2652,7 +2688,9 @@
 
 static int spgemm(padne_ctx *ctx, const padne_csr *X, const padne_csr *Y, padne_csr **C, const SlotRows *y_slots = nullptr,
                   SlotRows *keep_slots = nullptr, const std::function<int()> *while_counting = nullptr,
-                  const std::function<int()> *while_multiplying = nullptr) {
+                  const std::function<int()> *while_multiplying = nullptr, int with_dinv = 0) {
+    const int unfolded = ctx->opt.force_amg_unfolded;
+    const bool fold_dinv = !(unfolded & 2), fold_pend_pipe = !(unfolded & 4), fold_ends = !(unfolded & 8);
     const int *y_begin = y_slots != nullptr ? y_slots->begin : Y->rowptr;
     const int *y_end = y_slots != nullptr ? y_slots->end : Y->rowptr + 1;
     const int *y_cols = y_slots != nullptr ? (const int *)y_slots->key + 1 : Y->cols;
@@ -2721,6 +2759,8 @@
     int *row_begin = nullptr;
     PADNE_TRY(sc.alloc(&key, (size_t)n_slots + 4));
     PADNE_TRY(sc.alloc(&val, (size_t)n_slots + 4));
+    int *row_end = nullptr;
+    if (fold_ends && keep_slots != nullptr) PADNE_TRY(sc.alloc(&row_end, (size_t)(n > 0 ? n : 1)));
     if (n > 0) {
         const double avg = (double)n_slots / (double)n;
         const size_t dense_lds = (size_t)Y->n_cols * 9 + 16;
@@ -2728,28 +2768,31 @@
             (void)hipFuncSetAttribute((const void *)spgemm_rows_dense, hipFuncAttributeMaxDynamicSharedMemorySize,
                                       (int)dense_lds);
             hipLaunchKernelGGL(spgemm_rows_dense, dim3(n), dim3(256), dense_lds, s, (int)Y->n_cols, X->rowptr, X->cols,
-                               X->vals, y_begin, y_cols, y_vals, y_end, y_cs, slot_ptr, key, val, row_len, 0);
+                               X->vals, y_begin, y_cols, y_vals, y_end, y_cs, slot_ptr, key, val, row_len, 0, (const int *)nullptr,
+                               (const int *)nullptr, row_end);
         } else if (avg <= 24.0) {
+            int *pend = nullptr, *pend_count = nullptr;
             {
                 PADNE_TRY(sc.alloc(&row_begin, (size_t)n + 1));
-                if (y_cs == 1)
-                    hipLaunchKernelGGL((spgemm_rows_lds_pipe<12, 9, 4, 1>), dim3(nblk(n, 128)), dim3(128), 0, s, n, X->rowptr, X->cols,
-                                       X->vals, y_begin, y_cols, y_vals, y_end, slot_ptr, key, val, row_len, row_begin);
-                else
-                    hipLaunchKernelGGL((spgemm_rows_lds_pipe<12, 9, 4, 2>), dim3(nblk(n, 128)), dim3(128), 0, s, n, X->rowptr, X->cols,
-                                       X->vals, y_begin, y_cols, y_vals, y_end, slot_ptr, key, val, row_len, row_begin);
-            }
-            {
-                const int *place = row_begin != nullptr ? row_begin : slot_ptr;
-                int *pend = nullptr, *pend_count = nullptr;
                 PADNE_TRY(sc.alloc(&pend, (size_t)n));
                 PADNE_TRY(sc.alloc(&pend_count, 1));
                 PADNE_HIP_CHECK(hipMemsetAsync(pend_count, 0, sizeof(int), s));
-                hipLaunchKernelGGL(collect_pending_rows, dim3(nblk(n)), dim3(256), 0, s, n, (const int *)row_len, pend, pend_count);
+                int *pend_w = fold_pend_pipe ? pend : nullptr;
+                if (y_cs == 1)
+                    hipLaunchKernelGGL((spgemm_rows_lds_pipe<12, 9, 4, 1>), dim3(nblk(n, 128)), dim3(128), 0, s, n, X->rowptr, X->cols,
+                                       X->vals, y_begin, y_cols, y_vals, y_end, slot_ptr, key, val, row_len, row_begin, row_end, pend_w, pend_count);
+                else
+                    hipLaunchKernelGGL((spgemm_rows_lds_pipe<12, 9, 4, 2>), dim3(nblk(n, 128)), dim3(128), 0, s, n, X->rowptr, X->cols,
+                                       X->vals, y_begin, y_cols, y_vals, y_end, slot_ptr, key, val, row_len, row_begin, row_end, pend_w, pend_count);
+            }
+            {
+                const int *place = row_begin != nullptr ? row_begin : slot_ptr;
+                if (!fold_pend_pipe)
+                    hipLaunchKernelGGL(collect_pending_rows, dim3(nblk(n)), dim3(256), 0, s, n, (const int *)row_len, pend, pend_count);
                 hipLaunchKernelGGL((spgemm_rows_lanes<1024, 512, 64, true>), dim3(256), dim3(256), 0, s, n, X->rowptr, X->cols, X->vals, y_begin,
-                                   y_cols, y_vals, y_end, y_cs, place, key, val, row_len, (const int *)pend, (const int *)pend_count);
+                                   y_cols, y_vals, y_end, y_cs, place, key, val, row_len, (const int *)pend, (const int *)pend_count, row_end);
                 hipLaunchKernelGGL(spgemm_rows_redo, dim3(nblk(n, 128)), dim3(128), 0, s, n, X->rowptr, X->cols, X->vals,
-                                   y_begin, y_cols, y_vals, y_end, y_cs, place, key, val, row_len);
+                                   y_begin, y_cols, y_vals, y_end, y_cs, place, key, val, row_len, row_end);
             }
         } else if (avg <= 256.0) {
             const unsigned gw = (unsigned)std::min<long long>(((long long)n + 3) / 4, 16384);
@@ -2763,47 +2806,57 @@
                 if (x_avg > 0.0 && x_avg <= 14.0 && avg <= 48.0) {
                     unsigned gs = (unsigned)std::min<long long>(((long long)n + 15) / 16, 16384);
                     hipLaunchKernelGGL((spgemm_rows_lanes<128, 32, 16, false>), dim3(gs), dim3(256), 0, s, n, X->rowptr, X->cols, X->vals,
-                                       y_begin, y_cols, y_vals, y_end, y_cs, slot_ptr, key, val, row_len);
+                                       y_begin, y_cols, y_vals, y_end, y_cs, slot_ptr, key, val, row_len, (const int *)nullptr,
+                                       (const int *)nullptr, row_end);
                 } else {
                     unsigned gs = (unsigned)std::min<long long>(((long long)n + 7) / 8, 16384);
                     hipLaunchKernelGGL((spgemm_rows_lanes<256, 64, 32, false>), dim3(gs), dim3(256), 0, s, n, X->rowptr, X->cols, X->vals,
-                                       y_begin, y_cols, y_vals, y_end, y_cs, slot_ptr, key, val, row_len);
+                                       y_begin, y_cols, y_vals, y_end, y_cs, slot_ptr, key, val, row_len, (const int *)nullptr,
+                                       (const int *)nullptr, row_end);
                 }
                 hipLaunchKernelGGL(collect_pending_rows, dim3(nblk(n)), dim3(256), 0, s, n, (const int *)row_len, pend, pend_count);
                 hipLaunchKernelGGL((spgemm_rows_lanes<256, 128, 64, true>), dim3(gl), dim3(256), 0, s, n, X->rowptr, X->cols, X->vals,
                                    y_begin, y_cols, y_vals, y_end, y_cs, slot_ptr, key, val, row_len, (const int *)pend,
-                                   (const int *)pend_count);
+                                   (const int *)pend_count, row_end);
             } else {
                 hipLaunchKernelGGL((spgemm_rows_lanes<512, 256, 64, false>), dim3(gw), dim3(256), 0, s, n, X->rowptr, X->cols, X->vals,
-                                   y_begin, y_cols, y_vals, y_end, y_cs, slot_ptr, key, val, row_len);
+                                   y_begin, y_cols, y_vals, y_end, y_cs, slot_ptr, key, val, row_len, (const int *)nullptr,
+                                   (const int *)nullptr, row_end);
                 hipLaunchKernelGGL(collect_pending_rows, dim3(nblk(n)), dim3(256), 0, s, n, (const int *)row_len, pend, pend_count);
             }
             hipLaunchKernelGGL((spgemm_rows_lanes<1024, 512, 64, true>), dim3(std::min(gl, 1024u)), dim3(256), 0, s, n, X->rowptr, X->cols,
                                X->vals, y_begin, y_cols, y_vals, y_end, y_cs, slot_ptr, key, val, row_len, (const int *)pend,
-                               (const int *)pend_count);
+                               (const int *)pend_count, row_end);
             if (dense_lds <= 150 * 1024) {
                 (void)hipFuncSetAttribute((const void *)spgemm_rows_dense, hipFuncAttributeMaxDynamicSharedMemorySize,
                                           (int)dense_lds);
                 hipLaunchKernelGGL(spgemm_rows_dense, dim3(std::min(n, 1024)), dim3(256), dense_lds, s, (int)Y->n_cols, X->rowptr, X->cols,
                                    X->vals, y_begin, y_cols, y_vals, y_end, y_cs, slot_ptr, key, val, row_len, 1, (const int *)pend,
-                                   (const int *)pend_count);
+                                   (const int *)pend_count, row_end);
             }
             hipLaunchKernelGGL(spgemm_rows_redo, dim3(nblk(n, 128)), dim3(128), 0, s, n, X->rowptr, X->cols, X->vals,
-                               y_begin, y_cols, y_vals, y_end, y_cs, slot_ptr, key, val, row_len);
+                               y_begin, y_cols, y_vals, y_end, y_cs, slot_ptr, key, val, row_len, row_end);
         } else {
             hipLaunchKernelGGL(spgemm_rows, dim3(nblk(n, 128)), dim3(128), 0, s, n, X->rowptr, X->cols, X->vals,
-                               y_begin, y_cols, y_vals, y_end, y_cs, slot_ptr, key, val, row_len);
+                               y_begin, y_cols, y_vals, y_end, y_cs, slot_ptr, key, val, row_len, row_end);
         }
     }
     PADNE_HIP_CHECK(hipGetLastError());
     if (while_multiplying != nullptr && keep_slots != nullptr) PADNE_TRY((*while_multiplying)());
     if (keep_slots != nullptr) {
         keep_slots->release();
-        int *end = (int *)pool_alloc(ctx, sizeof(int) * (size_t)(n > 0 ? n : 1));
-        if (end == nullptr) return PADNE_E_NOMEM;
         int *first = row_begin != nullptr ? row_begin : slot_ptr;
-        if (n > 0) hipLaunchKernelGGL(slot_row_ends, dim3(nblk(n)), dim3(256), 0, s, n, (const int *)first, row_len, end);
-        PADNE_HIP_CHECK(hipGetLastError());
+        int *end = row_end;
+        if (end == nullptr) {
+            end = (int *)pool_alloc(ctx, sizeof(int) * (size_t)(n > 0 ? n : 1));
+            if (end == nullptr) return PADNE_E_NOMEM;
+            if (n > 0) hipLaunchKernelGGL(slot_row_ends, dim3(nblk(n)), dim3(256), 0, s, n, (const int *)first, row_len, end);
+            PADNE_HIP_CHECK(hipGetLastError());
+        } else {
+            sc.disown(row_end);
+            keep_slots->len = row_len;
+            sc.disown(row_len);
+        }
         keep_slots->ctx = ctx;
         keep_slots->n_rows = n;
         keep_slots->n_cols = Y->n_cols;
@@ -2821,7 +2874,8 @@
     }
     auto trampoline = [](void *f) -> int { return (*static_cast<const std::function<int()> *>(f))(); };
     return csr_from_slots(ctx, n, Y->n_cols, row_begin != nullptr ? row_begin : slot_ptr, key, val, row_len, C,
-                          while_multiplying != nullptr ? +trampoline : nullptr, const_cast<std::function<int()> *>(while_multiplying));
+                          while_multiplying != nullptr ? +trampoline : nullptr, const_cast<std::function<int()> *>(while_multiplying),
+                          fold_dinv ? with_dinv : 0);
 }
 
 __global__ void slot_row_lengths(int n, const int *__restrict__ begin, const int *__restrict__ end, int *__restrict__ len) {
@@ -2890,8 +2944,12 @@
     hipStream_t s = ctx->stream;
     const int n = (int)A->n_rows;
     Scratch sc(ctx);
-    int *len = nullptr;
-    PADNE_TRY(sc.alloc(&len, (size_t)n + 1));
+    const int *len = ap.len;
+    int *len_tmp = nullptr;
+    if (len == nullptr) {
+        PADNE_TRY(sc.alloc(&len_tmp, (size_t)n + 1));
+        len = len_tmp;
+    }
     struct CsrDrop { void operator()(padne_csr *m) const { if (m) padne_csr_destroy(m); } };
     std::unique_ptr<padne_csr, CsrDrop> w_owner(new padne_csr());
     padne_csr *W = w_owner.get();
@@ -2906,7 +2964,7 @@
     W->cols = (int32_t *)pool_alloc(ctx, sizeof(int32_t) * ((size_t)n_slots + kPadNnz));
     W->vals32 = (float *)pool_alloc(ctx, sizeof(float) * ((size_t)n_slots + kPadNnz));
     if (!W->rowptr || !W->cols || !W->vals32) return PADNE_E_NOMEM;
-    hipLaunchKernelGGL(slot_row_lengths, dim3(nblk(n)), dim3(256), 0, s, n, ap.begin, ap.end, len);
+    if (len_tmp != nullptr) hipLaunchKernelGGL(slot_row_lengths, dim3(nblk(n)), dim3(256), 0, s, n, ap.begin, ap.end, len_tmp);
     PADNE_HIP_CHECK(hipGetLastError());
     PADNE_TRY(exclusive_scan_i32_async(ctx, len, W->rowptr, n));
     unsigned gw = nblk(((long long)n + 63) / 64, 4);
@@ -3220,9 +3278,9 @@
             padne_csr ap_shape;
             ap_shape.n_rows = ap_rows.n_rows;
             ap_shape.n_cols = ap_rows.n_cols;
-            rc = spgemm(ctx, L.R, &ap_shape, &Ac, &ap_rows, nullptr, nullptr, &queue_side);
+            rc = spgemm(ctx, L.R, &ap_shape, &Ac, &ap_rows, nullptr, nullptr, &queue_side, want_f32 ? 2 : 1);
         } else {
-            rc = spgemm(ctx, L.R, AP, &Ac, nullptr, nullptr, nullptr, &queue_side);
+            rc = spgemm(ctx, L.R, AP, &Ac, nullptr, nullptr, nullptr, &queue_side, want_f32 ? 2 : 1);
         }
         if (rc == PADNE_OK && !side_queued) rc = queue_side();
         if (rc != PADNE_OK && two) (void)hipStreamSynchronize(aux->stream);
@@ -3233,6 +3291,7 @@
             std::swap(to.ctx, from.ctx);
             std::swap(to.begin, from.begin);
             std::swap(to.end, from.end);
+            std::swap(to.len, from.len);
             std::swap(to.key, from.key);
             std::swap(to.val, from.val);
             to.n_rows = from.n_rows;
@@ -3806,13 +3865,13 @@
             padne_csr ap_shape;
             ap_shape.n_rows = ap_rows.n_rows;
             ap_shape.n_cols = ap_rows.n_cols;
-            rc = spgemm(ctx, Lr.R, &ap_shape, &Ac, &ap_rows);
+            rc = spgemm(ctx, Lr.R, &ap_shape, &Ac, &ap_rows, nullptr, nullptr, nullptr, 1);
             if (rc == PADNE_OK && want_f32 && A->dinv != nullptr && (ctx->opt.amg_w == 2 || (ctx->opt.amg_w == 1 && lvl == 0))) {
                 rc = build_w_operator(ctx, A, Lr.P, ap_rows, ap_rows.n_slots, Lr.jac, &Lr.W, 0, lvl == 0);
                 if (rc == PADNE_OK) Lr.W->n_cols = P_ext->n_cols;
             }
         } else {
-            rc = spgemm(ctx, Lr.R, AP, &Ac);
+            rc = spgemm(ctx, Lr.R, AP, &Ac, nullptr, nullptr, nullptr, nullptr, 1);
         }
         ap_rows.release();
         padne_csr_destroy(P_ext);
diff --git a/padne_amd/csrc/assemble.hip b/padne_amd/csrc/assemble.hip
--- a/padne_amd/csrc/assemble.hip
+++ b/padne_amd/csrc/assemble.hip
@@ -1488,11 +1488,13 @@
 __global__ __launch_bounds__(256) void compact_rows(long long n_rows, const int *__restrict__ slot_ptr,
                                                     const int *__restrict__ rowptr, const long long *__restrict__ key,
                                                     const double *__restrict__ val, int *__restrict__ cols,
-                                                    double *__restrict__ vals, const int rpw) {
+                                                    double *__restrict__ vals, const int rpw,
+                                                    double *__restrict__ dinv = nullptr, float *__restrict__ dinv32 = nullptr) {
     __shared__ int rp_all[4][65];
     __shared__ int sp_all[4][65];
+    __shared__ int dg_all[4][64];
     const int lane = threadIdx.x & 63, w = threadIdx.x >> 6;
-    int *rp = rp_all[w], *sp = sp_all[w];
+    int *rp = rp_all[w], *sp = sp_all[w], *dg = dg_all[w];
     const long long n_wt = (n_rows + rpw - 1) / rpw;
     for (long long wt = (long long)blockIdx.x * 4 + w; wt < n_wt; wt += (long long)gridDim.x * 4) {
         const long long r0 = wt * rpw;
@@ -1500,6 +1502,7 @@
         if (lane <= nr) rp[lane] = rowptr[r0 + lane];
         if (lane < nr) sp[lane] = slot_ptr[r0 + lane];
         if (lane == 0 && nr == 64) rp[64] = rowptr[r0 + 64];
+        if (dinv != nullptr) dg[lane] = 0;
         asm volatile("s_waitcnt lgkmcnt(0)" ::: "memory");
         __builtin_amdgcn_wave_barrier();
         const int d0 = rp[0], d1 = rp[nr];
@@ -1510,8 +1513,25 @@
                 if (rp[mid] <= k) lo = mid; else hi = mid;
             }
             const int src = sp[lo] + (k - rp[lo]);
-            cols[k] = (int)(key[src] >> 32);
-            vals[k] = val[src];
+            const int c = (int)(key[src] >> 32);
+            const double v = val[src];
+            cols[k] = c;
+            vals[k] = v;
+            if (dinv != nullptr && (long long)c == r0 + lo) {
+                const double d = 1.0 / (0.0 + v);
+                dinv[r0 + lo] = d;
+                if (dinv32 != nullptr) dinv32[r0 + lo] = (float)d;
+                dg[lo] = 1;
+            }
+        }
+        if (dinv != nullptr) {
+            asm volatile("s_waitcnt lgkmcnt(0)" ::: "memory");
+            __builtin_amdgcn_wave_barrier();
+            if (lane < nr && dg[lane] == 0) {
+                const double d = 1.0 / 0.0;
+                dinv[r0 + lane] = d;
+                if (dinv32 != nullptr) dinv32[r0 + lane] = (float)d;
+            }
         }
         asm volatile("" ::: "memory");
         __builtin_amdgcn_wave_barrier();
@@ -1945,7 +1965,8 @@
 }
 
 int csr_from_slots(padne_ctx *ctx, long long n_rows, long long n_cols, const int *slot_ptr, const long long *key,
-                   const double *val, const int *row_len, padne_csr **out, int (*while_scanning)(void *), void *while_scanning_arg) {
+                   const double *val, const int *row_len, padne_csr **out, int (*while_scanning)(void *), void *while_scanning_arg,
+                   int with_dinv) {
     hipStream_t s = ctx->stream;
     Scratch sc(ctx);
     int *rowptr_tmp = nullptr;
@@ -1973,10 +1994,18 @@
     PADNE_TRY(csr_alloc(ctx, n_rows, n_cols, nnz, &m));
     hipError_t e = hipMemcpyAsync(m->rowptr, rowptr_tmp, sizeof(int32_t) * (size_t)(n_rows + 1),
                                   hipMemcpyDeviceToDevice, s);
+    if (with_dinv > 0 && n_rows > 0 && n_rows <= n_cols) {
+        m->dinv = (double *)pool_alloc(ctx, sizeof(double) * (size_t)n_rows);
+        if (with_dinv > 1) m->dinv32 = (float *)pool_alloc(ctx, sizeof(float) * (size_t)n_rows);
+        if (m->dinv == nullptr || (with_dinv > 1 && m->dinv32 == nullptr)) {
+            padne_csr_destroy(m);
+            return PADNE_E_NOMEM;
+        }
+    }
     if (e == hipSuccess && n_rows > 0) {
         const int rpw = compact_rows_per_wave(n_rows, nnz);
         hipLaunchKernelGGL(compact_rows, dim3(std::min(nblk((n_rows + rpw - 1) / rpw, 4), 65536u)), dim3(256), 0, s, n_rows, slot_ptr,
-                           m->rowptr, key, val, m->cols, m->vals, rpw);
+                           m->rowptr, key, val, m->cols, m->vals, rpw, m->dinv, m->dinv32);
         e = hipGetLastError();
     }
     if (e != hipSuccess) {
diff --git a/padne_amd/csrc/capi.hip b/padne_amd/csrc/capi.hip
--- a/padne_amd/csrc/capi.hip
+++ b/padne_amd/csrc/capi.hip
@@ -52,6 +52,7 @@
         o->force_transpose_cursors = has(f, "transpose_cursors") != nullptr;
         o->force_xhist_small = has(f, "xhist_small") != nullptr;
         o->force_relabel_lanes = has(f, "relabel_lanes") != nullptr;
+        if (const char *w = has(f, "amg_unfolded")) o->force_amg_unfolded = w[12] == ':' ? atoi(w + 13) & 31 : 31;
         if (const char *w = has(f, "spgemm_split")) o->force_spgemm_split = w[12] == ':' ? atoll(w + 13) : 30000;
     }
     if (const char *e = getenv("PADNE_POOL_GUARD")) {
diff --git a/padne_amd/csrc/common.hpp b/padne_amd/csrc/common.hpp
--- a/padne_amd/csrc/common.hpp
+++ b/padne_amd/csrc/common.hpp
@@ -121,6 +121,7 @@
     bool force_relabel_lanes = false;
     bool force_xhist_small = false;
     long long force_spgemm_split = 0;
+    int force_amg_unfolded = 0;
     bool verbose_amg = false, verbose_xw = false, verbose_pool = false;
     int pool_guard = -1;
 };
@@ -338,7 +339,7 @@
 int sort_slots_exact(padne_ctx *ctx, long long n_rows, const int *slot_ptr, long long *key, double *val, int *row_len_scratch);
 int csr_from_slots(padne_ctx *ctx, long long n_rows, long long n_cols, const int *slot_ptr, const long long *key,
                    const double *val, const int *row_len, padne_csr **out,
-                   int (*while_scanning)(void *) = nullptr, void *while_scanning_arg = nullptr);
+                   int (*while_scanning)(void *) = nullptr, void *while_scanning_arg = nullptr, int with_dinv = 0);
 int csr_from_exact_slots(padne_ctx *ctx, long long n_rows, long long n_cols, long long nnz, const int *slot_ptr,
                          const long long *key, const double *val, padne_csr **out);
 
```

New measurement: 32.31 solves/s. Within noise of the previous version (-0.4%).
